# kzampog/cilantro

Hardware: AMD Instinct MI355X
Metric: ICP corr. pairs/sec (+ iterations/sec), synthetic uniform clouds (higher is better)
Workload: dtype f32 search / f64 accumulate+solve

## Files before the change

### cilantro_amd/capi.py

```python
import ctypes as C
import os

_HERE = os.path.dirname(os.path.abspath(__file__))
LIB_PATH = os.environ.get("CILHIP_LIB_PATH") or os.path.join(_HERE, "lib", "libcilantro_hip.so")

OK, ERR_INVALID, ERR_HIP, ERR_UNSUPPORTED, ERR_NO_DEVICE = 0, -1, -2, -3, -4
MEM_HOST, MEM_DEVICE = 0, 1
METRIC_POINT_TO_POINT, METRIC_COMBINED = 0, 1
SUMS_LEN = 48
NONE_IDX = 0xFFFFFFFF

SYMBOLS = [
    "cilhip_create", "cilhip_destroy", "cilhip_last_error", "cilhip_set_stream", "cilhip_synchronize",
    "cilhip_set_target", "cilhip_set_source", "cilhip_set_source_normals", "cilhip_get_means", "cilhip_set_color_features", "cilhip_share_target", "cilhip_find_correspondences",
    "cilhip_get_nn", "cilhip_get_correspondences", "cilhip_estimate_point_to_point",
    "cilhip_estimate_combined", "cilhip_estimate_affine", "cilhip_icp_default_params", "cilhip_icp_run", "cilhip_icp_begin",
    "cilhip_icp_partial_sums", "cilhip_icp_apply_sums", "cilhip_icp_state", "cilhip_compute_residuals",
    "cilhip_get_grid_info", "cilhip_get_last_timing", "cilhip_enable_kernel_timing", "cilhip_prepare_source", "cilhip_get_last_run_forms", "cilhip_get_last_warm_iterations", "cilhip_get_last_matches_origin", "cilhip_get_matches_transform", "cilhip_get_last_form_timing", "cilhip_get_last_iteration_timing", "cilhip_get_last_run_trace", "cilhip_estimate_combined_two_sets", "cilhip_icp_run_two_sets", "cilhip_set_pair_weight_callback", "cilhip_kmeans_set_pruning", "cilhip_get_tie_count", "cilhip_get_tie_rule_stats", "cilhip_get_tie_order_info", "cilhip_build_tie_order", "cilhip_tie_order_create", "cilhip_tie_order_destroy", "cilhip_tie_order_tables", "cilhip_load_tie_order", "cilhip_multi_create", "cilhip_multi_destroy", "cilhip_multi_last_error", "cilhip_multi_context", "cilhip_multi_set_clouds", "cilhip_multi_icp_run", "cilhip_multi_repartitions", "cilhip_multi_last_host_time", "cilhip_multi_set_slab_slack", "cilhip_multi_shard_sizes", "cilhip_rank_comm_unique_id", "cilhip_rank_comm_prepare", "cilhip_rank_comm_init", "cilhip_rank_comm_destroy", "cilhip_icp_iterate_ranked", "cilhip_get_last_allreduce_timing", "cilhip_get_last_host_enqueue_time", "cilhip_set_slab_guard", "cilhip_get_slab_violation", "cilhip_get_slab_violation_state",
    "cilhip_set_option", "cilhip_option_count", "cilhip_option_info", "cilhip_set_option_id", "cilhip_get_option", "cilhip_get_last_timing2", "cilhip_set_shard_info", "cilhip_icp_partial_keys",
    "cilhip_icp_sums_from_keys", "cilhip_icp_order_keys", "cilhip_icp_sums_from_ordered_keys", "cilhip_debug_counters", "cilhip_kmeans3f", "cilhip_kmeans3f_assign", "cilhip_kmeans3f_ex", "cilhip_kmeans3f_assign_ex", "cilhip_kmeans_shard_create", "cilhip_kmeans_shard_destroy", "cilhip_kmeans_shard_maxabs", "cilhip_kmeans_scale_exponent", "cilhip_kmeans_shard_assign", "cilhip_kmeans_shard_farthest", "cilhip_kmeans_shard_move_point", "cilhip_kmeans_shard_labels",
    "cilhip_plane_ransac3f", "cilhip_plane_score3f", "cilhip_plane_fit3f", "cilhip_transform_ransac3f", "cilhip_transform_score3f", "cilhip_transform_fit3f", "cilhip_knn3f", "cilhip_knn_set_tie_rule", "cilhip_normals_knn3f", "cilhip_normals_radius3f", "cilhip_radius_search3f",
]


PAIR_WEIGHT_FN = C.CFUNCTYPE(None, C.c_void_p, C.POINTER(C.c_uint64), C.POINTER(C.c_uint64), C.POINTER(C.c_float), C.c_size_t,
                             C.POINTER(C.c_float), C.POINTER(C.c_float))


class IcpParams(C.Structure):
    _fields_ = [
        ("metric", C.c_int), ("w_p2p", C.c_float), ("w_p2pl", C.c_float), ("max_iter", C.c_size_t),
        ("conv_tol", C.c_float), ("max_opt_iter", C.c_size_t), ("opt_conv_tol", C.c_float),
        ("max_sq_dist", C.c_float),
    ]


class IcpResult(C.Structure):
    _fields_ = [
        ("T", C.c_float * 16), ("iterations", C.c_size_t), ("last_delta_norm", C.c_float),
        ("last_ncorr", C.c_size_t),
    ]


class GridInfo(C.Structure):
    _fields_ = [
        ("nx", C.c_int), ("ny", C.c_int), ("nz", C.c_int), ("cell", C.c_float),
        ("origin", C.c_float * 3), ("n_cells", C.c_size_t), ("avg_occupancy", C.c_double),
        ("build_ms", C.c_double),
    ]


class OptionInfo(C.Structure):
    _fields_ = [("id", C.c_int), ("key", C.c_char_p), ("default_value", C.c_double), ("min_value", C.c_double), ("max_value", C.c_double),
                ("doc", C.c_char_p)]


class TieOrderInfo(C.Structure):
    _fields_ = [("loaded", C.c_int), ("builds", C.c_int), ("build_ms", C.c_double), ("pending", C.c_size_t)]


class PlaneModel(C.Structure):
    _fields_ = [
        ("normal", C.c_float * 3), ("offset", C.c_float), ("iterations", C.c_size_t), ("n_inliers", C.c_size_t),
        ("target_reached", C.c_int), ("device_ms", C.c_double),
    ]


class TransformModel(C.Structure):
    _fields_ = [
        ("T", C.c_float * 16), ("iterations", C.c_size_t), ("n_inliers", C.c_size_t), ("have_model", C.c_int),
        ("target_reached", C.c_int), ("device_ms", C.c_double),
    ]


_lib = None


def load():
    global _lib
    if _lib is not None:
        return _lib
    if not os.path.exists(LIB_PATH):
        raise RuntimeError(
            f"{LIB_PATH} is missing: the HIP extension has not been built "
            "(run `python -m cilantro_amd.build` / `__graft_entry__.build()`). There is no CPU fallback."
        )
    try:
        import torch
    except ImportError:
        pass
    L = C.CDLL(LIB_PATH)
    vp, f32p, f64p = C.c_void_p, C.c_void_p, C.c_void_p
    L.cilhip_create.argtypes = [C.POINTER(vp), C.c_int]
    L.cilhip_destroy.argtypes = [vp]
    L.cilhip_destroy.restype = None
    L.cilhip_last_error.argtypes = [vp]
    L.cilhip_last_error.restype = C.c_char_p
    L.cilhip_set_stream.argtypes = [vp, vp]
    L.cilhip_synchronize.argtypes = [vp]
    L.cilhip_set_target.argtypes = [vp, f32p, f32p, C.c_size_t, C.c_int]
    L.cilhip_set_source.argtypes = [vp, f32p, C.c_size_t, C.c_int]
    L.cilhip_set_source_normals.argtypes = [vp, f32p, C.c_int]
    L.cilhip_get_means.argtypes = [vp, f32p, f32p]
    L.cilhip_find_correspondences.argtypes = [vp, f32p, C.c_float, C.POINTER(C.c_size_t)]
    L.cilhip_get_nn.argtypes = [vp, vp, f32p, C.c_int]
    L.cilhip_get_correspondences.argtypes = [vp, vp, vp, f32p, C.c_size_t, C.POINTER(C.c_size_t)]
    L.cilhip_estimate_point_to_point.argtypes = [vp, f32p, f64p, C.POINTER(C.c_int)]
    L.cilhip_estimate_combined.argtypes = [vp, C.c_float, C.c_float, C.c_size_t, C.c_float, f32p, f64p,
                                           f64p, C.POINTER(C.c_int)]
    L.cilhip_estimate_affine.argtypes = [vp, C.c_float, C.c_float, C.c_int, f32p, f64p, f64p, C.POINTER(C.c_size_t), C.POINTER(C.c_int)]
    L.cilhip_icp_default_params.argtypes = [C.POINTER(IcpParams)]
    L.cilhip_icp_default_params.restype = None
    L.cilhip_icp_run.argtypes = [vp, C.POINTER(IcpParams), f32p, C.POINTER(IcpResult)]
    L.cilhip_icp_begin.argtypes = [vp, C.POINTER(IcpParams), f32p, f32p]
    L.cilhip_icp_partial_sums.argtypes = [vp, f64p]
    L.cilhip_icp_apply_sums.argtypes = [vp, f64p]
    L.cilhip_icp_state.argtypes = [vp, C.POINTER(IcpResult)]
    L.cilhip_compute_residuals.argtypes = [vp, C.c_int, C.c_float, C.c_float, f32p, f32p, C.c_int]
    L.cilhip_get_grid_info.argtypes = [vp, C.POINTER(GridInfo)]
    L.cilhip_get_last_timing.argtypes = [vp, C.POINTER(C.c_double), C.POINTER(C.c_double), C.POINTER(C.c_int)]
    L.cilhip_enable_kernel_timing.argtypes = [vp, C.c_int]
    L.cilhip_set_option.argtypes = [vp, C.c_char_p, C.c_double]
    L.cilhip_share_target.argtypes = [vp, vp]
    L.cilhip_option_count.argtypes = []
    L.cilhip_option_info.argtypes = [C.c_int]
    L.cilhip_option_info.restype = C.POINTER(OptionInfo)
    L.cilhip_set_option_id.argtypes = [vp, C.c_int, C.c_double]
    L.cilhip_get_option.argtypes = [vp, C.c_char_p, C.POINTER(C.c_double)]
    L.cilhip_set_shard_info.argtypes = [vp, C.c_uint64, f32p, f32p]
    L.cilhip_icp_partial_keys.argtypes = [vp, vp]
    L.cilhip_debug_counters.argtypes = [vp, vp]
    L.cilhip_kmeans3f.argtypes = [C.c_int, f32p, C.c_size_t, C.c_int, f32p, C.c_size_t, C.c_size_t, C.c_float, vp, C.POINTER(C.c_size_t)]
    L.cilhip_kmeans3f_assign.argtypes = [C.c_int, f32p, C.c_size_t, C.c_int, f32p, C.c_size_t, vp]
    L.cilhip_kmeans3f_ex.argtypes = [C.c_int, f32p, C.c_size_t, C.c_int, f32p, C.c_size_t, C.c_size_t, C.c_float, C.c_int, vp, C.POINTER(C.c_size_t)]
    L.cilhip_kmeans3f_assign_ex.argtypes = [C.c_int, f32p, C.c_size_t, C.c_int, f32p, C.c_size_t, C.c_int, vp]
    L.cilhip_kmeans_shard_create.argtypes = [C.c_int, f32p, C.c_size_t, C.c_int, C.c_size_t, C.c_uint64, C.POINTER(C.c_void_p)]
    L.cilhip_kmeans_shard_destroy.argtypes = [vp]
    L.cilhip_kmeans_shard_destroy.restype = None
    L.cilhip_kmeans_shard_maxabs.argtypes = [vp, C.POINTER(C.c_float)]
    L.cilhip_kmeans_scale_exponent.argtypes = [C.c_double, C.c_size_t]
    L.cilhip_kmeans_shard_assign.argtypes = [vp, vp, C.c_int, C.c_int, vp, C.POINTER(C.c_uint64)]
    L.cilhip_kmeans_shard_farthest.argtypes = [vp, C.c_uint32, vp, C.POINTER(C.c_uint64)]
    L.cilhip_kmeans_shard_move_point.argtypes = [vp, C.c_uint64, C.c_uint32, vp]
    L.cilhip_kmeans_shard_labels.argtypes = [vp, vp]
    L.cilhip_plane_ransac3f.argtypes = [C.c_int, f32p, C.c_size_t, C.c_int, vp, C.c_uint64, C.c_float, C.c_size_t, C.c_size_t,
                                        C.c_int, C.POINTER(PlaneModel), vp, vp]
    L.cilhip_plane_score3f.argtypes = [C.c_int, f32p, C.c_size_t, C.c_int, f32p, C.c_size_t, C.c_float, vp]
    L.cilhip_plane_fit3f.argtypes = [C.c_int, f32p, C.c_size_t, C.c_int, f32p]
    L.cilhip_transform_ransac3f.argtypes = [C.c_int, f32p, f32p, C.c_size_t, C.c_int, vp, C.c_uint64, C.c_float, C.c_size_t, C.c_size_t,
                                            C.c_int, C.POINTER(TransformModel), vp, vp]
    L.cilhip_transform_score3f.argtypes = [C.c_int, f32p, f32p, C.c_size_t, C.c_int, f32p, C.c_size_t, C.c_float, vp]
    L.cilhip_transform_fit3f.argtypes = [C.c_int, f32p, f32p, C.c_size_t, C.c_int, f32p]
    L.cilhip_knn3f.argtypes = [C.c_int, f32p, C.c_size_t, f32p, C.c_size_t, C.c_int, C.c_size_t, C.c_float, vp, vp, vp]
    L.cilhip_normals_radius3f.argtypes = [C.c_int, f32p, C.c_size_t, C.c_int, C.c_float, f32p, f32p, f32p]
    L.cilhip_radius_search3f.argtypes = [C.c_int, f32p, C.c_size_t, f32p, C.c_size_t, C.c_int, C.c_float, vp, vp, vp, C.c_size_t,
                                         C.POINTER(C.c_size_t)]
    L.cilhip_normals_knn3f.argtypes = [C.c_int, f32p, C.c_size_t, C.c_int, C.c_size_t, C.c_float, f32p, f32p, f32p]
    L.cilhip_icp_sums_from_keys.argtypes = [vp, vp, f64p]
    L.cilhip_icp_order_keys.argtypes = [vp, vp, vp]
    L.cilhip_icp_sums_from_ordered_keys.argtypes = [vp, vp, vp, f64p]
    L.cilhip_get_last_timing2.argtypes = [vp, C.POINTER(C.c_double), C.POINTER(C.c_double)]
    L.cilhip_prepare_source.argtypes = [vp, C.c_void_p, C.c_int, C.POINTER(C.c_double)]
    L.cilhip_get_last_run_forms.argtypes = [vp, C.POINTER(C.c_int), C.POINTER(C.c_int)]
    L.cilhip_get_last_warm_iterations.argtypes = [vp, C.POINTER(C.c_int)]
    L.cilhip_set_color_features.argtypes = [vp, vp, vp, C.c_int]
    L.cilhip_get_last_matches_origin.argtypes = [vp, C.POINTER(C.c_int)]
    L.cilhip_get_matches_transform.argtypes = [vp, vp]
    L.cilhip_get_last_form_timing.argtypes = [vp, C.c_int, C.POINTER(C.c_double), C.POINTER(C.c_int)]
    L.cilhip_estimate_combined_two_sets.argtypes = [vp, vp, C.c_float, C.c_float, C.c_size_t, C.c_float, vp, C.POINTER(C.c_int)]
    L.cilhip_icp_run_two_sets.argtypes = [vp, C.c_float, vp, C.c_float, C.POINTER(IcpParams), vp, C.POINTER(IcpResult)]
    L.cilhip_set_pair_weight_callback.argtypes = [vp, PAIR_WEIGHT_FN, vp]
    L.cilhip_get_tie_count.argtypes = [vp, vp, C.c_float, C.POINTER(C.c_size_t)]
    L.cilhip_get_last_iteration_timing.argtypes = [vp, C.c_int, C.POINTER(C.c_int), vp, vp]
    L.cilhip_get_tie_rule_stats.argtypes = [vp, C.POINTER(C.c_size_t), C.POINTER(C.c_size_t)]
    L.cilhip_get_tie_order_info.argtypes = [vp, C.POINTER(TieOrderInfo)]
    L.cilhip_build_tie_order.argtypes = [vp]
    L.cilhip_tie_order_create.argtypes = [vp, C.c_size_t, C.POINTER(C.c_void_p)]
    L.cilhip_tie_order_tables.argtypes = [vp, vp, vp, vp, C.c_size_t, C.POINTER(C.c_size_t), C.POINTER(C.c_int)]
    L.cilhip_tie_order_destroy.argtypes = [vp]
    L.cilhip_tie_order_destroy.restype = None
    L.cilhip_load_tie_order.argtypes = [vp, vp, vp]
    L.cilhip_multi_create.argtypes = [C.POINTER(vp), C.POINTER(C.c_int), C.c_int]
    L.cilhip_multi_destroy.argtypes = [vp]; L.cilhip_multi_destroy.restype = None
    L.cilhip_multi_last_error.argtypes = [vp]; L.cilhip_multi_last_error.restype = C.c_char_p
    L.cilhip_multi_context.argtypes = [vp, C.c_int]; L.cilhip_multi_context.restype = vp
    L.cilhip_multi_set_clouds.argtypes = [vp, vp, vp, C.c_size_t, vp, C.c_size_t, C.c_float, C.c_int, vp]
    L.cilhip_multi_icp_run.argtypes = [vp, C.POINTER(IcpParams), vp, C.c_int, C.POINTER(IcpResult)]
    L.cilhip_multi_repartitions.argtypes = [vp]
    L.cilhip_multi_set_slab_slack.argtypes = [vp, C.c_float]
    L.cilhip_multi_shard_sizes.argtypes = [vp, C.c_int, C.POINTER(C.c_size_t), C.POINTER(C.c_size_t)]
    L.cilhip_rank_comm_unique_id.argtypes = [vp]
    L.cilhip_rank_comm_init.argtypes = [vp, vp, C.c_int, C.c_int]
    L.cilhip_rank_comm_prepare.argtypes = [vp]
    L.cilhip_rank_comm_destroy.argtypes = [vp]
    L.cilhip_icp_iterate_ranked.argtypes = [vp, C.c_int]
    L.cilhip_get_last_allreduce_timing.argtypes = [vp, C.POINTER(C.c_double), C.POINTER(C.c_int)]
    L.cilhip_get_last_host_enqueue_time.argtypes = [vp, C.POINTER(C.c_double)]
    L.cilhip_get_last_run_trace.argtypes = [vp, C.c_int, C.POINTER(C.c_int), C.POINTER(C.c_uint), C.POINTER(C.c_uint), C.POINTER(C.c_float), C.POINTER(C.c_float), C.POINTER(C.c_int)]
    L.cilhip_set_slab_guard.argtypes = [vp, C.c_int, C.c_float, f32p, f32p, f32p]
    L.cilhip_get_slab_violation.argtypes = [vp, C.POINTER(C.c_int)]
    L.cilhip_get_slab_violation_state.argtypes = [vp, C.POINTER(C.c_int), vp]
    for name in SYMBOLS:
        fn = getattr(L, name)
        if name not in ("cilhip_destroy", "cilhip_last_error", "cilhip_icp_default_params", "cilhip_option_info"):
            fn.restype = C.c_int
    _lib = L
    return L


class CilhipError(RuntimeError):
    def __init__(self, code, msg):
        super().__init__(f"cilhip error {code}: {msg}")
        self.code = code

# ... 9 lines not shown
```

### cilantro_amd/csrc/c_api.hip

```cpp
#include "../../include/cilantro_hip/c_api.h"

#include <hip/hip_runtime.h>

#include <algorithm>
#include <atomic>
#include <chrono>
#include <condition_variable>
#include <mutex>
#include <cmath>
#include <cstddef>
#include <cstdio>
#include <cstring>
#include <new>
#include <string>
#include <thread>
#include <vector>

#include "internal.hpp"

using namespace cilhip;

struct TargetShare { int refs = 0; std::vector<void*> allocs; };

struct cilhip_ctx {
  int device = 0;
  TargetShare* tshare = nullptr;
  hipStream_t own_stream = nullptr;
  hipStream_t stream = nullptr;
  std::string err;

  bool has_target = false;
  GridDev grid{};
  bool has_normals = false;
  double grid_occ = 0.0;
  size_t grid_cells = 0;
  double build_ms = 0.0;
  float dst_mean[3] = {0, 0, 0};
  uint32_t index_offset = 0;
  bool partial_target = false;
  uint32_t* d_inv_perm = nullptr;

  bool has_source = false;
  uint32_t ns = 0;
  float* d_src_xyz = nullptr;
  float4* d_src_sorted = nullptr;
  SortWorkspace sort_ws;
  uint32_t tile_aux_cap = 0;
  uint2* d_tiles = nullptr;
  float4* d_tile_center = nullptr;
  int* d_tile_box = nullptr;
  float tile_axes[9] = {0, 0, 0, 0, 0, 0, 0, 0, 0};
  unsigned long long* d_defer_mask = nullptr;
  uint32_t* d_defer_flag = nullptr;
  uint32_t* d_unproven = nullptr;
  bool warm_banned = false;
  Feedback* h_feedback = nullptr;
  Feedback* d_feedback = nullptr;
  unsigned int run_tag = 0;
  bool far_mode = true;
  int last_fused_iters = 0, last_two_pass_iters = 0, last_warm_iters = 0;
  int run_calls = 0;
  bool run_warm_on = false;
  unsigned int run_judged = 0;
  std::vector<unsigned char> iter_form;
  std::vector<unsigned char> trace_form;
  double form_ms[5] = {0, 0, 0, 0, 0};
  int form_n[5] = {0, 0, 0, 0, 0};
  int warm_start = 1;
  uint32_t* d_dbg = nullptr;
  uint4* d_trace = nullptr;
  uint32_t ntiles = 0;
  int tiled = 1;
  bool src_sorted = false;
  float sort_T[16];
  float src_mean[3] = {0, 0, 0};
  float* d_src_nrm = nullptr;
  float4* d_src_nrm_sorted = nullptr;
  uint32_t* d_nn_pos = nullptr;
  float* d_nn_d2 = nullptr;
  float4* d_warm_rec = nullptr;
  bool rec_valid = false;
  bool src3_valid = false;
  float* d_nn_lb = nullptr;
  bool lb_fresh = false;
  bool warm_forecast = true;
  int tie_rule = 2;
  uint2* d_tief_leaf_slot = nullptr;
  uint4* d_tief_nodes = nullptr;
  int tief_builds = 0;
  uint2* d_tie_leaf_slot = nullptr;
  uint4* d_tie_nodes = nullptr;
  unsigned int* d_tie_counters = nullptr;
  unsigned int* d_ticket = nullptr;
  int group_lanes = -1;
  double wait_us = 0.0;
  bool feat_warm = true;
  bool affine_device_loop = true;
  bool fused_epilogue = false;
  unsigned int tie_counters_host[4] = {0, 0, 0, 0};
  bool tie_counters_fresh = false;
  double tie_build_ms = 0.0;
  int tie_builds = 0;
  bool rev_tie_aware = false;
  uint2* d_rev_tie_leaf_slot = nullptr;
  uint4* d_rev_tie_nodes = nullptr;
  size_t rev_tie_nodes_cap = 0;
  bool rev_tie_valid = false;
  float rev_tie_T[16];
  int rev_tie_builds = 0;
  float warm_extra = 0.0625f;
  bool pair_records = true;
  void* rank_comm = nullptr; int rank_comm_size = 0; double* d_rank_sums = nullptr;
  bool tile_records = true;
  float warm_enter = 0.15f;
  float warm_thresh = 0.0f;
  int warm_strikes = 0;
  float src_center[3] = {0, 0, 0}, src_half[3] = {0, 0, 0};
  float* d_safe2 = nullptr;
  int cw_point_kind = 0, cw_plane_kind = 0;
  float cw_point_sigma = 1.0f, cw_plane_sigma = 1.0f;
  cilhip_pair_weight_fn weight_fn = nullptr;
  void* weight_user = nullptr;
  float* d_wtab = nullptr;
// ... 54 lines not shown

  cilhip_icp_params run_prm{};
  bool run_active = false;
  int guard_axis = -1;
  float guard_slack = 0.0f, guard_center[3] = {0, 0, 0}, guard_half[3] = {0, 0, 0}, guard_T[16] = {0};
  float run_src_mean[3] = {0, 0, 0};

  bool kernel_timing = false;
  int timing_stride = 1;
  std::vector<unsigned int> timed_iter;
  std::vector<float> timed_ms;
  double last_loop_ms = 0.0, last_search_ms = 0.0, last_acc_ms = 0.0;
  int last_search_launches = 0;
  size_t run_nev = 0;
  std::vector<hipEvent_t> ev, ev_acc;
  std::vector<hipEvent_t> ev_ar;
  size_t run_nar = 0;
  double last_allreduce_ms = 0.0; int last_allreduce_n = 0;
  double run_enqueue_us = 0.0; int run_enqueue_iters = 0;

};

#define CK(ctx, call)                                                                                   \
  do {                                                                                                  \
    hipError_t e_ = (call);                                                                             \
    if (e_ != hipSuccess) {                                                                             \
      (ctx)->err = std::string(#call) + ": " + hipGetErrorString(e_);                                   \
      return CILHIP_ERR_HIP;                                                                            \
    }                                                                                                   \
  } while (0)

static int fail(cilhip_ctx* c, int code, const char* msg) {
  if (c) c->err = msg;
  return code;
}

static const float kIdentity[16] = {1, 0, 0, 0, 0, 1, 0, 0, 0, 0, 1, 0, 0, 0, 0, 1};
namespace cilhip {
hipStream_t ctx_stream(const cilhip_ctx* c) { return c->stream; }
double ctx_wait_us(const cilhip_ctx* c) { return c->wait_us; }
}

static void drop_src_grid(cilhip_ctx* c) {
  if (c->has_src_grid) { free_grid(c->src_grid); c->has_src_grid = false; }
  if (c->d_src_safe2) { (void)hipFree(c->d_src_safe2); c->d_src_safe2 = nullptr; }
  if (c->d_grid_to_sorted) { (void)hipFree(c->d_grid_to_sorted); c->d_grid_to_sorted = nullptr; }
  if (c->d_src_rgb_grid) { (void)hipFree(c->d_src_rgb_grid); c->d_src_rgb_grid = nullptr; }
}
static void drop_matches(cilhip_ctx* c) { c->have_nn = false; c->d2_stale = false; c->pending_matches = false; c->matches_origin = 0; }
static void drop_rev_tie_tables(cilhip_ctx* c) {
  if (c->d_rev_tie_leaf_slot) { (void)hipFree(c->d_rev_tie_leaf_slot); c->d_rev_tie_leaf_slot = nullptr; }
  if (c->d_rev_tie_nodes) { (void)hipFree(c->d_rev_tie_nodes); c->d_rev_tie_nodes = nullptr; }
  c->rev_tie_nodes_cap = 0; c->rev_tie_valid = false; c->rev_tie_aware = false;
}
static void target_ptr_free(cilhip_ctx* c, const void* p) {
  if (!p) return;
  if (c->tshare && std::find(c->tshare->allocs.begin(), c->tshare->allocs.end(), p) != c->tshare->allocs.end()) return;
  (void)hipFree(const_cast<void*>(p));
}
static void release_target_share(cilhip_ctx* c) {
  if (!c->tshare) return;
  if (--c->tshare->refs == 0) {
    for (void* p : c->tshare->allocs) (void)hipFree(p);
    delete c->tshare;
  }
  c->tshare = nullptr;
}
static void drop_feat_tie_tables(cilhip_ctx* c) {
  if (c->d_tief_leaf_slot) { (void)hipFree(c->d_tief_leaf_slot); c->d_tief_leaf_slot = nullptr; }
  if (c->d_tief_nodes) { (void)hipFree(c->d_tief_nodes); c->d_tief_nodes = nullptr; }
}
static void drop_tie_tables(cilhip_ctx* c) {
  target_ptr_free(c, c->d_tie_leaf_slot); c->d_tie_leaf_slot = nullptr;
  target_ptr_free(c, c->d_tie_nodes); c->d_tie_nodes = nullptr;
}
static void release_target(cilhip_ctx* c) {
  if (c->has_target) {
    target_ptr_free(c, c->grid.pts); target_ptr_free(c, c->grid.nrm); target_ptr_free(c, c->grid.pn); target_ptr_free(c, c->grid.cell_start);
    c->grid.pts = nullptr; c->grid.nrm = nullptr; c->grid.pn = nullptr; c->grid.cell_start = nullptr;
    c->has_target = false;
  }
  target_ptr_free(c, c->d_inv_perm); c->d_inv_perm = nullptr;
  target_ptr_free(c, c->d_safe2); c->d_safe2 = nullptr;
  drop_tie_tables(c);
  drop_feat_tie_tables(c);
  release_target_share(c);
}

extern "C" {

int cilhip_create(cilhip_ctx** out, int device) {
  if (!out) return CILHIP_ERR_INVALID;
  *out = nullptr;
  int ndev = 0;
  if (hipGetDeviceCount(&ndev) != hipSuccess || ndev <= 0) return CILHIP_ERR_NO_DEVICE;
  if (device < 0 || device >= ndev) return CILHIP_ERR_INVALID;
  cilhip_ctx* c = new (std::nothrow) cilhip_ctx();
  if (!c) return CILHIP_ERR_HIP;
  c->device = device;
  if (hipSetDevice(device) != hipSuccess || hipStreamCreateWithFlags(&c->own_stream, hipStreamNonBlocking) != hipSuccess) {
    delete c;
    return CILHIP_ERR_HIP;
  }
  c->stream = c->own_stream;
  if (hipMalloc(&c->d_state, sizeof(IcpState)) != hipSuccess || hipMalloc(&c->d_count, sizeof(unsigned long long)) != hipSuccess ||
      hipMalloc(&c->d_defer_flag, sizeof(uint32_t)) != hipSuccess || hipMemset(c->d_defer_flag, 0, sizeof(uint32_t)) != hipSuccess ||
      hipMalloc(&c->d_unproven, 128 * sizeof(uint32_t)) != hipSuccess || hipMemset(c->d_unproven, 0, 128 * sizeof(uint32_t)) != hipSuccess ||
      hipMalloc(&c->d_ticket, sizeof(unsigned int)) != hipSuccess || hipMemset(c->d_ticket, 0, sizeof(unsigned int)) != hipSuccess ||
      hipHostMalloc(&c->h_feedback, sizeof(Feedback), hipHostMallocMapped | hipHostMallocCoherent) != hipSuccess ||
      hipHostGetDevicePointer(reinterpret_cast<void**>(&c->d_feedback), c->h_feedback, 0) != hipSuccess ||
      hipMalloc(&c->d_trace, RUN_TRACE_CAP * sizeof(uint4)) != hipSuccess || hipMemset(c->d_trace, 0, RUN_TRACE_CAP * sizeof(uint4)) != hipSuccess ||
      hipMalloc(&c->d_stage, REDUCE_STAGE_DOUBLES * sizeof(double)) != hipSuccess || hipMalloc(&c->d_sums, 3 * SUMS_MAX * sizeof(double)) != hipSuccess) {
    delete c;
    return CILHIP_ERR_HIP;
  }
  if (hipMemset(c->d_state, 0, sizeof(IcpState)) != hipSuccess) { delete c; return CILHIP_ERR_HIP; }
  c->d_tie_counters = reinterpret_cast<unsigned int*>(reinterpret_cast<char*>(c->d_state) + offsetof(IcpState, tie_counters));
  memcpy(c->sort_T, kIdentity, sizeof(kIdentity));
  memcpy(c->nn_T, kIdentity, sizeof(kIdentity));
  *out = c;
  return CILHIP_OK;
}

static void free_source(cilhip_ctx* c) {
  drop_rev_tie_tables(c);
  if (c->d_src_xyz) (void)hipFree(c->d_src_xyz);
  if (c->d_src_sorted) (void)hipFree(c->d_src_sorted);
  if (c->d_nn_pos) (void)hipFree(c->d_nn_pos);
  if (c->d_nn_d2) (void)hipFree(c->d_nn_d2);
  if (c->d_warm_rec) { (void)hipFree(c->d_warm_rec); c->d_warm_rec = nullptr; }
  if (c->d_nn_lb) { (void)hipFree(c->d_nn_lb); c->d_nn_lb = nullptr; }
  c->src3_valid = false; c->lb_fresh = false;
  c->rec_valid = false;
  if (c->d_out_idx) (void)hipFree(c->d_out_idx);
  if (c->d_out_d2) (void)hipFree(c->d_out_d2);
  free_sort_workspace(c->sort_ws);
  c->tile_aux_cap = 0;
  if (c->d_tile_box) (void)hipFree(c->d_tile_box);
  if (c->d_src_nrm) (void)hipFree(c->d_src_nrm);
  if (c->d_src_nrm_sorted) (void)hipFree(c->d_src_nrm_sorted);
  c->d_src_nrm = nullptr; c->d_src_nrm_sorted = nullptr;
  if (c->d_src_rgb) (void)hipFree(c->d_src_rgb);
  if (c->d_src_rgb_sorted) (void)hipFree(c->d_src_rgb_sorted);
  c->d_src_rgb = nullptr; c->d_src_rgb_sorted = nullptr;
  if (c->d_defer_mask) (void)hipFree(c->d_defer_mask);
  if (c->d_keys) (void)hipFree(c->d_keys);
  c->d_keys = nullptr;
  if (c->d_own_order) (void)hipFree(c->d_own_order);
  c->d_own_order = nullptr;
  c->d_tiles = nullptr; c->d_tile_center = nullptr; c->d_tile_box = nullptr; c->ntiles = 0; c->d_defer_mask = nullptr;
  c->d_src_xyz = nullptr; c->d_src_sorted = nullptr; c->d_nn_pos = nullptr; c->d_nn_d2 = nullptr;
  c->d_out_idx = nullptr; c->d_out_d2 = nullptr;
  drop_src_grid(c);
  if (c->d_src_inv) { (void)hipFree(c->d_src_inv); c->d_src_inv = nullptr; }
  if (c->d_grid_to_sorted) { (void)hipFree(c->d_grid_to_sorted); c->d_grid_to_sorted = nullptr; }
  c->has_source = false; c->src_sorted = false; drop_matches(c); c->ns = 0;
  c->have_pairs = false; c->pairs.count = 0;
  c->far_mode = true;
  c->warm_banned = false;
}

void cilhip_destroy(cilhip_ctx* c) {
  if (!c) return;
  (void)hipSetDevice(c->device);
  (void)hipStreamSynchronize(c->stream);
  (void)cilhip_rank_comm_destroy(c);
  free_source(c);
  release_target(c);
  if (c->d_ticket) (void)hipFree(c->d_ticket);
  if (c->d_wtab) (void)hipFree(c->d_wtab);
  if (c->d_wtab_in) (void)hipFree(c->d_wtab_in);
  if (c->d_dst_rgb) (void)hipFree(c->d_dst_rgb);
  if (c->d_dst_rgb_sorted) (void)hipFree(c->d_dst_rgb_sorted);
  if (c->d_state) (void)hipFree(c->d_state);
  if (c->d_state_id) (void)hipFree(c->d_state_id);
  free_pairs(c->pairs);
  if (c->d_partials) (void)hipFree(c->d_partials);
  if (c->d_sel_state) (void)hipFree(c->d_sel_state);
  if (c->d_winner) (void)hipFree(c->d_winner);
  if (c->d_count) (void)hipFree(c->d_count);
  if (c->d_dbg) (void)hipFree(c->d_dbg);
  if (c->d_trace) (void)hipFree(c->d_trace);
  if (c->d_defer_flag) (void)hipFree(c->d_defer_flag);
  if (c->d_unproven) (void)hipFree(c->d_unproven);
  if (c->d_rev_pos) (void)hipFree(c->d_rev_pos);
  if (c->d_rev_d2) (void)hipFree(c->d_rev_d2);
  if (c->h_feedback) (void)hipHostFree(c->h_feedback);
  if (c->d_stage) (void)hipFree(c->d_stage);
  if (c->d_sums) (void)hipFree(c->d_sums);
  for (auto e : c->ev) (void)hipEventDestroy(e);
  for (auto e : c->ev_acc) (void)hipEventDestroy(e);
  for (auto e : c->ev_ar) (void)hipEventDestroy(e);

  if (c->own_stream) (void)hipStreamDestroy(c->own_stream);
  delete c;
}

const char* cilhip_last_error(const cilhip_ctx* c) { return c ? c->err.c_str() : "null context"; }

int cilhip_set_stream(cilhip_ctx* c, void* s) {
  if (!c) return CILHIP_ERR_INVALID;
  (void)hipSetDevice(c->device);
  (void)hipStreamSynchronize(c->stream);
  c->stream = s ? (hipStream_t)s : c->own_stream;
  return CILHIP_OK;
}

int cilhip_synchronize(cilhip_ctx* c) {
  if (!c) return CILHIP_ERR_INVALID;
  CK(c, hipSetDevice(c->device));
  CK(c, hipStreamSynchronize(c->stream));
  return CILHIP_OK;
}

namespace {
struct OptionRow { cilhip_option_info_t info; double (*get)(const cilhip_ctx*); };
#define OPT(ID, KEY, DEF, LO, HI, DOC, EXPR) {{ID, KEY, DEF, LO, HI, DOC}, [](const cilhip_ctx* c) -> double { return (double)(EXPR); }}
const OptionRow g_options[] = {
  OPT(CILHIP_OPT_FUSED, "fused", 0, 0, 1, "1 = one per-lane search+accumulate kernel per iteration; 0 = search kernel + streaming accumulation (or the LDS tiles)", c->fused),
  OPT(CILHIP_OPT_INLIER_FRACTION, "inlier_fraction", 1, 0, 1, "CorrespondenceSearchKDTree::setInlierFraction: keep that fraction of the correspondences, nearest first", c->inlier_fraction),
  OPT(CILHIP_OPT_ONE_TO_ONE, "one_to_one", 0, 0, 1, "setOneToOne: a target point keeps only its nearest source point", c->one_to_one),
  OPT(CILHIP_OPT_TILED, "tiled", 1, 0, 2, "LDS-tiled search: 0 = never, 1 = when the cloud fills the chip with full tiles, 2 = always", c->tiled),
  OPT(CILHIP_OPT_WARM_START, "warm_start", 1, 0, 2, "warm-started iterations (margin proof): 0 = never, 1 = when the loop is near alignment, 2 = from the second iteration on", c->warm_start),
  OPT(CILHIP_OPT_WARM_FORECAST, "warm_forecast", 1, 0, 1, "the cold kernels' forecast gates the warm-started form (0: the step alone; tests)", c->warm_forecast),
  OPT(CILHIP_OPT_FUSED_EPILOGUE, "fused_epilogue", 0, 0, 1, "stage-1 reduction + epilogue as one launch behind a device-scope fence (bitwise equal, measured slower; A/B)", c->fused_epilogue),
  OPT(CILHIP_OPT_GROUP_SEARCH, "group_search", -1, -1, 64, "lanes per query of the cooperative global-memory search: -1 = the loop decides, 0 = never, 4 / 8 / 16 / 32 / 64", c->group_lanes),
  OPT(CILHIP_OPT_TIE_RULE, "tie_rule", 2, 0, 2, "exactly equidistant nearest points: 0 = lowest index, 1 = the reference's kd-tree order (tables up front), 2 = the same, tables when a tie is first met", c->tie_rule),
  OPT(CILHIP_OPT_WARM_EXTRA_FRACTION, "warm_extra_fraction", 0.0625, 1e-9, 1, "room (fraction of a cell) of the ball a warm-started iteration searches a listed query in", c->warm_extra),
  OPT(CILHIP_OPT_PAIR_RECORDS, "pair_records", 1, 0, 1, "streaming accumulation gathers a match's point and normal from one 32-byte record (A/B)", c->pair_records),
  OPT(CILHIP_OPT_TILE_RECORDS, "tile_records", 1, 0, 1, "the accumulating tile kernel writes the warm-started form's match records itself (A/B)", c->tile_records),
  OPT(CILHIP_OPT_WARM_ENTER_FRACTION, "warm_enter_fraction", 0.15, 1e-9, 1e9, "the warm-started form is entered once an update moves no source point by more than this fraction of a cell", c->warm_enter),
  OPT(CILHIP_OPT_POINT_WEIGHT_EVALUATOR, "point_weight_evaluator", 0, 0, 2, "combined metric, point-to-point terms: 0 = UnityWeightEvaluator, 1 = DistanceEvaluator, 2 = RBFKernelWeightEvaluator", c->cw_point_kind),
  OPT(CILHIP_OPT_PLANE_WEIGHT_EVALUATOR, "plane_weight_evaluator", 0, 0, 2, "combined metric, point-to-plane terms: 0 = Unity, 1 = Identity (distance), 2 = RBF kernel", c->cw_plane_kind),
  OPT(CILHIP_OPT_POINT_WEIGHT_SIGMA, "point_weight_sigma", 1, 1e-30, 1e30, "sigma of the RBF evaluator of the point-to-point terms", c->cw_point_sigma),
  OPT(CILHIP_OPT_PLANE_WEIGHT_SIGMA, "plane_weight_sigma", 1, 1e-30, 1e30, "sigma of the RBF evaluator of the point-to-plane terms", c->cw_plane_sigma),
  OPT(CILHIP_OPT_TILE_ACCUMULATION, "tile_accumulation", 1, 0, 2, "first Gauss-Newton step accumulated inside the LDS tiles: 0 = never, 1 = unless the source is far from alignment, 2 = always", (c->tile_acc ? (c->tile_acc_adaptive ? 1 : 2) : 0)),
  OPT(CILHIP_OPT_SEARCH_DIRECTION, "search_direction", 0, 0, 2, "CorrespondenceSearchDirection: 0 = SECOND_TO_FIRST, 1 = FIRST_TO_SECOND, 2 = BOTH", c->search_dir),
  OPT(CILHIP_OPT_FEATURE_NORMAL_WEIGHT, "feature_normal_weight", 0, 0, 1e30, "PointNormalFeaturesAdaptor's normal weight (> 0: the search runs on 6-D features)", c->normal_weight),
  OPT(CILHIP_OPT_FEATURE_KIND, "feature_kind", 0, 0, 2, "second feature block: 0 = normals (follow the transform), 1 = colours (do not), 2 = normals + colours (9-D)", c->feature_kind),
  OPT(CILHIP_OPT_FEATURE_COLOR_WEIGHT, "feature_color_weight", 0, 0, 1e30, "PointNormalColorFeaturesAdaptor's colour weight (feature_kind 2)", c->color_weight),
  OPT(CILHIP_OPT_SYMMETRIC_METRIC, "symmetric_metric", 1, 0, 1, "source normals, when set, switch the combined metric to the symmetric objective", c->symmetric),
  OPT(CILHIP_OPT_TRANSFORM_MODE, "transform_mode", 0, 0, 1, "ICP instance family: 0 = rigid, 1 = affine", c->transform_mode),
  OPT(CILHIP_OPT_REQUIRE_RECIPROCALITY, "require_reciprocality", 0, 0, 1, "setRequireReciprocality (search_direction BOTH)", c->reciprocal),
  OPT(CILHIP_OPT_CELL_OCCUPANCY, "cell_occupancy", 1, 1e-3, 1e6, "target points per grid cell the next cilhip_set_target aims at", c->cell_occupancy),
  OPT(CILHIP_OPT_REFINED_OCCUPANCY_FACTOR, "refined_occupancy_factor", 3, 1, 64, "how much denser than that a grid that had to be refined (surface, clusters) may stay", c->refined_occupancy),
  OPT(CILHIP_OPT_KERNEL_TIMING, "kernel_timing", 0, 0, 1, "hipEvents around the search / accumulation kernels (cilhip_enable_kernel_timing)", c->kernel_timing),
  OPT(CILHIP_OPT_KERNEL_TIMING_STRIDE, "kernel_timing_stride", 1, 1, 4096, "with kernel timing on: iterations 0..2 and every stride-th one carry events", c->timing_stride),
  OPT(CILHIP_OPT_REVERSE_WARM_START, "reverse_warm_start", 1, 0, 1, "device-resident FIRST_TO_SECOND / BOTH loops: reverse searches after the first start from the previous reverse matches (margin test over the source; A/B)", c->reverse_warm),
  OPT(CILHIP_OPT_FEATURE_WARM_START, "feature_warm_start", 1, 0, 1, "feature adaptors (SECOND_TO_FIRST loops): searches warm-started from the previous matches once the loop moves little (margin test with the feature distance; A/B)", c->feat_warm),
  OPT(CILHIP_OPT_AFFINE_DEVICE_LOOP, "affine_device_loop", 1, 0, 1, "affine classes: 1 = device-resident loop (one-pass moments, solve in the epilogue kernel), 0 = host-driven loop (three passes + host solve; A/B)", c->affine_device_loop),
};
#undef OPT
constexpr int N_OPTIONS = (int)(sizeof(g_options) / sizeof(g_options[0]));
static_assert(N_OPTIONS == CILHIP_OPT_COUNT, "one table row per enum cilhip_option value, in the enum's order");
}

int cilhip_option_count(void) { return N_OPTIONS; }
const cilhip_option_info_t* cilhip_option_info(int id) { return (id >= 0 && id < N_OPTIONS) ? &g_options[id].info : nullptr; }
int cilhip_set_option_id(cilhip_ctx* c, cilhip_option id, double value) {
  if (!c) return CILHIP_ERR_INVALID;
  if ((int)id < 0 || (int)id >= N_OPTIONS) return fail(c, CILHIP_ERR_INVALID, "set_option_id: unknown option");
  return cilhip_set_option(c, g_options[(int)id].info.key, value);
}
int cilhip_get_option(cilhip_ctx* c, const char* key, double* value) {
  if (!c || !key || !value) return CILHIP_ERR_INVALID;
  for (int i = 0; i < N_OPTIONS; ++i)
    if (!strcmp(key, g_options[i].info.key)) { *value = g_options[i].get(c); return CILHIP_OK; }
  return fail(c, CILHIP_ERR_INVALID, "get_option: unknown key");
}

int cilhip_set_option(cilhip_ctx* c, const char* key, double value) {
  if (!c || !key) return CILHIP_ERR_INVALID;
  if (value != value) return fail(c, CILHIP_ERR_INVALID, "set_option: the value is not a number");
  if (!strcmp(key, "fused")) { c->fused = value != 0.0; return CILHIP_OK; }
  if (!strcmp(key, "inlier_fraction")) { if (c->inlier_fraction != value && c->pending_matches) drop_matches(c); c->inlier_fraction = value; return CILHIP_OK; }
  if (!strcmp(key, "one_to_one")) { if (c->one_to_one != (value != 0.0) && c->pending_matches) drop_matches(c); c->one_to_one = value != 0.0; return CILHIP_OK; }
  if (!strcmp(key, "tiled")) { c->tiled = (int)value; return CILHIP_OK; }
  if (!strcmp(key, "warm_start")) { c->warm_start = (int)value; return CILHIP_OK; }
  if (!strcmp(key, "warm_forecast")) { c->warm_forecast = value != 0.0; return CILHIP_OK; }
  if (!strcmp(key, "fused_epilogue")) { c->fused_epilogue = value != 0.0; return CILHIP_OK; }
  if (!strcmp(key, "reverse_warm_start")) { c->reverse_warm = value != 0.0; return CILHIP_OK; }
  if (!strcmp(key, "feature_warm_start")) { c->feat_warm = value != 0.0; return CILHIP_OK; }
  if (!strcmp(key, "affine_device_loop")) { c->affine_device_loop = value != 0.0; return CILHIP_OK; }
  if (!strcmp(key, "group_search")) {
    if (value != -1.0 && value != 0.0 && value != 4.0 && value != 8.0 && value != 16.0 && value != 32.0 && value != 64.0)
      return fail(c, CILHIP_ERR_INVALID, "group_search: -1 (the loop decides), 0 (never), or 4, 8, 16, 32, 64 lanes per query");
    c->group_lanes = (int)value;
    return CILHIP_OK;
  }
  if (!strcmp(key, "tie_rule")) {
    if (value != 0.0 && value != 1.0 && value != 2.0)
      return fail(c, CILHIP_ERR_INVALID, "tie_rule: 0 (lowest index), 1 (the reference's kd-tree order, tables built up front) or 2 (the same, tables built when a tie is first met)");
    if (((int)value != 0) != (c->tie_rule != 0)) drop_matches(c);
    c->tie_rule = (int)value;
    return CILHIP_OK;
  }
  if (!strcmp(key, "warm_extra_fraction")) {
    if (!(value > 0.0 && value <= 1.0)) return fail(c, CILHIP_ERR_INVALID, "warm_extra_fraction: in (0, 1]");
    c->warm_extra = (float)value;
    return CILHIP_OK;
  }
  if (!strcmp(key, "pair_records")) { c->pair_records = value != 0.0; return CILHIP_OK; }
  if (!strcmp(key, "tile_records")) { c->tile_records = value != 0.0; return CILHIP_OK; }
  if (!strcmp(key, "warm_enter_fraction")) {
    if (!(value > 0.0)) return fail(c, CILHIP_ERR_INVALID, "warm_enter_fraction: > 0 (fraction of a grid cell)");
    c->warm_enter = (float)value;
    return CILHIP_OK;
  }
  if (!strcmp(key, "point_weight_evaluator") || !strcmp(key, "plane_weight_evaluator")) {
    if (value != 0.0 && value != 1.0 && value != 2.0) return fail(c, CILHIP_ERR_INVALID, "weight evaluator: 0 = Unity, 1 = Identity, 2 = RBF kernel");
    (key[1] == 'o' ? c->cw_point_kind : c->cw_plane_kind) = (int)value;
    return CILHIP_OK;
  }
  if (!strcmp(key, "point_weight_sigma") || !strcmp(key, "plane_weight_sigma")) {
    if (!(value > 0.0)) return fail(c, CILHIP_ERR_INVALID, "weight evaluator sigma must be positive");
    (key[1] == 'o' ? c->cw_point_sigma : c->cw_plane_sigma) = (float)value;
    return CILHIP_OK;
  }
  if (!strcmp(key, "tile_accumulation")) { c->tile_acc = value != 0.0; c->tile_acc_adaptive = value != 2.0; return CILHIP_OK; }
  if (!strcmp(key, "search_direction")) {
    if (value != 0.0 && value != 1.0 && value != 2.0) return fail(c, CILHIP_ERR_INVALID, "search_direction: 0 = SECOND_TO_FIRST, 1 = FIRST_TO_SECOND, 2 = BOTH");
    c->search_dir = (int)value; drop_matches(c); c->have_pairs = false;
    return CILHIP_OK;
  }
  if (!strcmp(key, "feature_normal_weight")) {
    if (!(value >= 0.0)) return fail(c, CILHIP_ERR_INVALID, "feature_normal_weight: >= 0 (0 = plain point features)");
    if (c->normal_weight != (float)value) drop_feat_tie_tables(c);
    c->normal_weight = (float)value; drop_matches(c); c->have_pairs = false;
    return CILHIP_OK;
  }
  if (!strcmp(key, "feature_kind")) {
    if (value != 0.0 && value != 1.0 && value != 2.0)
      return fail(c, CILHIP_ERR_INVALID, "feature_kind: 0 = normals (follow the transform), 1 = colours (do not), 2 = normals + colours (9-D)");
    if ((int)value != c->feature_kind) { drop_src_grid(c); drop_feat_tie_tables(c); }
    c->feature_kind = (int)value; drop_matches(c); c->have_pairs = false;
    return CILHIP_OK;
  }
  if (!strcmp(key, "feature_color_weight")) {
    if (!(value >= 0.0)) return fail(c, CILHIP_ERR_INVALID, "feature_color_weight: >= 0");
    if (c->color_weight != (float)value) drop_feat_tie_tables(c);
    c->color_weight = (float)value; drop_matches(c); c->have_pairs = false;
    return CILHIP_OK;
  }
  if (!strcmp(key, "symmetric_metric")) { c->symmetric = value != 0.0; return CILHIP_OK; }
  if (!strcmp(key, "transform_mode")) {
    if (value != 0.0 && value != 1.0) return fail(c, CILHIP_ERR_INVALID, "transform_mode: 0 = rigid, 1 = affine");
    c->transform_mode = (int)value;
    return CILHIP_OK;
  }
  if (!strcmp(key, "require_reciprocality")) { c->reciprocal = value != 0.0; drop_matches(c); c->have_pairs = false; return CILHIP_OK; }
  if (!strcmp(key, "cell_occupancy")) { c->cell_occupancy = value; return CILHIP_OK; }
  if (!strcmp(key, "refined_occupancy_factor")) {
    if (!(value >= 1.0 && value <= 64.0)) return fail(c, CILHIP_ERR_INVALID, "refined_occupancy_factor: in [1, 64]");
    c->refined_occupancy = value;
    return CILHIP_OK;
  }
  if (!strcmp(key, "kernel_timing")) { c->kernel_timing = value != 0.0; return CILHIP_OK; }
  if (!strcmp(key, "kernel_timing_stride")) {
    if (!(value >= 1.0 && value <= 4096.0)) return fail(c, CILHIP_ERR_INVALID, "kernel_timing_stride: 1 .. 4096");
    c->timing_stride = (int)value;
    return CILHIP_OK;
  }
  return fail(c, CILHIP_ERR_INVALID, "set_option: unknown key");
}

int cilhip_debug_counters(cilhip_ctx* c, uint32_t out[2]) {
  if (!c || !out) return CILHIP_ERR_INVALID;
  out[0] = out[1] = 0;
  if (!c->d_defer_mask || !c->ntiles) return CILHIP_OK;
  CK(c, hipSetDevice(c->device));
  if (!c->d_dbg) CK(c, hipMalloc(&c->d_dbg, 2 * sizeof(uint32_t)));
  launch_count_deferred(c->d_defer_mask, c->ntiles, c->d_dbg, c->stream);
  CK(c, hipMemcpyAsync(out, c->d_dbg, 2 * sizeof(uint32_t), hipMemcpyDeviceToHost, c->stream));
  CK(c, hipStreamSynchronize(c->stream));
#ifdef CILHIP_EXP_PHASE_CLOCKS
  cilhip::debug_dump_phase_clocks();
#endif
  return CILHIP_OK;
}

int cilhip_get_last_timing2(cilhip_ctx* c, double* search_ms, double* accumulate_ms) {
  if (!c) return CILHIP_ERR_INVALID;
  if (search_ms) *search_ms = c->last_search_ms;
  if (accumulate_ms) *accumulate_ms = c->last_acc_ms;
  return CILHIP_OK;
}

int cilhip_get_last_iteration_timing(cilhip_ctx* c, int cap, int* n, unsigned int* iteration, float* kernel_ms) {
  if (!c || !n || cap < 0) return CILHIP_ERR_INVALID;
  const size_t m = c->timed_ms.size() < c->timed_iter.size() ? c->timed_ms.size() : c->timed_iter.size();
  *n = (int)m;
  for (size_t k = 0; k < m && k < (size_t)cap; ++k) { if (iteration) iteration[k] = c->timed_iter[k]; if (kernel_ms) kernel_ms[k] = c->timed_ms[k]; }
  return CILHIP_OK;
}

int cilhip_get_last_form_timing(cilhip_ctx* c, int form, double* kernel_ms, int* launches) {
  if (!c || form < 0 || form > 4) return CILHIP_ERR_INVALID;
  if (kernel_ms) *kernel_ms = c->form_ms[form];
  if (launches) *launches = c->form_n[form];
  return CILHIP_OK;
}

int cilhip_get_last_run_trace(cilhip_ctx* c, int cap, int* n_out, unsigned int* unproven, unsigned int* listed, float* step, float* delta, int* form) {
  if (!c || !n_out || cap < 0) return CILHIP_ERR_INVALID;
  CK(c, hipSetDevice(c->device));
  IcpState hs;
  CK(c, hipMemcpyAsync(&hs, c->d_state, sizeof(hs), hipMemcpyDeviceToHost, c->stream));
  uint4 tr[RUN_TRACE_CAP];
  CK(c, hipMemcpyAsync(tr, c->d_trace, sizeof(tr), hipMemcpyDeviceToHost, c->stream));
  CK(c, hipStreamSynchronize(c->stream));
  const int n = std::min(std::min(hs.iterations, (int)RUN_TRACE_CAP), cap);
  for (int i = 0; i < n; ++i) {
    if (unproven) unproven[i] = tr[i].x;
    if (listed) listed[i] = tr[i].y;
    if (step) memcpy(&step[i], &tr[i].z, 4);
    if (delta) memcpy(&delta[i], &tr[i].w, 4);
    if (form) form[i] = (size_t)i < c->trace_form.size() ? (int)(c->trace_form[i] & 0x7f) : -1;
  }
  *n_out = n;
  return CILHIP_OK;
}

int cilhip_get_last_warm_iterations(cilhip_ctx* c, int* warm_iterations) {
  if (!c || !warm_iterations) return CILHIP_ERR_INVALID;
  *warm_iterations = c->last_warm_iters;
  return CILHIP_OK;
}

int cilhip_get_last_run_forms(cilhip_ctx* c, int* one_pass_iterations, int* two_pass_iterations) {
  if (!c) return CILHIP_ERR_INVALID;
  if (one_pass_iterations) *one_pass_iterations = c->last_fused_iters;
  if (two_pass_iterations) *two_pass_iterations = c->last_two_pass_iters;
  return CILHIP_OK;
}

int cilhip_enable_kernel_timing(cilhip_ctx* c, int on) {
  if (!c) return CILHIP_ERR_INVALID;
  c->kernel_timing = on != 0;
  return CILHIP_OK;
}

static int upload(cilhip_ctx* c, const float* src, size_t count, int mem, float** d_out) {
  *d_out = nullptr;
  CK(c, hipMalloc(d_out, (count ? count : 1) * sizeof(float)));
  if (count)
    CK(c, hipMemcpyAsync(*d_out, src, count * sizeof(float), mem == CILHIP_MEM_DEVICE ? hipMemcpyDeviceToDevice : hipMemcpyHostToDevice, c->stream));
  return CILHIP_OK;
}

int cilhip_set_target(cilhip_ctx* c, const float* xyz, const float* nrm, size_t n, int mem) {
  if (!c) return CILHIP_ERR_INVALID;
  if ((n && !xyz) || n >= 0xFFFFFFF0ull) return fail(c, CILHIP_ERR_INVALID, "set_target: bad cloud (null or >= 2^32-16 points)");
  CK(c, hipSetDevice(c->device));
  auto t0 = std::chrono::steady_clock::now();
  release_target(c);
  if (c->d_winner) { (void)hipFree(c->d_winner); c->d_winner = nullptr; }
  if (c->d_rev_pos) { (void)hipFree(c->d_rev_pos); c->d_rev_pos = nullptr; }
  if (c->d_rev_d2) { (void)hipFree(c->d_rev_d2); c->d_rev_d2 = nullptr; }
  float *d_xyz = nullptr, *d_nrm = nullptr;
  int rc = upload(c, xyz, 3 * n, mem, &d_xyz);
  if (rc) return rc;
  if (nrm) { rc = upload(c, nrm, 3 * n, mem, &d_nrm); if (rc) { (void)hipFree(d_xyz); return rc; } }
  GridBuildResult r{};
  double mean[3];
  hipError_t e = build_grid(d_xyz, d_nrm, (uint32_t)n, c->stream, &r, mean, c->cell_occupancy, c->refined_occupancy);
  (void)hipFree(d_xyz);
  if (d_nrm) (void)hipFree(d_nrm);
  if (e != hipSuccess) { c->err = std::string("build_grid: ") + hipGetErrorString(e); return CILHIP_ERR_HIP; }
  c->grid = r.grid; c->grid_occ = r.avg_occupancy; c->grid_cells = r.n_cells;
  c->warm_banned = false;
  c->dst_rgb_sorted_ok = false;
  if (c->d_dst_rgb) { (void)hipFree(c->d_dst_rgb); c->d_dst_rgb = nullptr; }
  if (c->d_dst_rgb_sorted) { (void)hipFree(c->d_dst_rgb_sorted); c->d_dst_rgb_sorted = nullptr; }
  c->has_normals = (nrm != nullptr);
  for (int i = 0; i < 3; ++i) c->dst_mean[i] = (float)mean[i];
  c->partial_target = false;
  c->has_target = true;
  c->src_sorted = false;
  drop_matches(c);
  c->have_pairs = false; c->pairs.count = 0;
  c->far_mode = true;
  c->build_ms = std::chrono::duration<double, std::milli>(std::chrono::steady_clock::now() - t0).count();
  return CILHIP_OK;
}

int cilhip_share_target(cilhip_ctx* c, cilhip_ctx* from) {
  if (!c || !from || c == from) return CILHIP_ERR_INVALID;
  if (!from->has_target) return fail(c, CILHIP_ERR_INVALID, "share_target: the other context has no target");
  if (c->device != from->device) return fail(c, CILHIP_ERR_INVALID, "share_target: the two contexts live on different devices");
  CK(c, hipSetDevice(c->device));
  CK(c, hipStreamSynchronize(from->stream));
  CK(c, hipStreamSynchronize(c->stream));
  release_target(c);
  if (c->d_winner) { (void)hipFree(c->d_winner); c->d_winner = nullptr; }
  if (c->d_rev_pos) { (void)hipFree(c->d_rev_pos); c->d_rev_pos = nullptr; }
  if (c->d_rev_d2) { (void)hipFree(c->d_rev_d2); c->d_rev_d2 = nullptr; }
  if (c->d_dst_rgb) { (void)hipFree(c->d_dst_rgb); c->d_dst_rgb = nullptr; }
  if (c->d_dst_rgb_sorted) { (void)hipFree(c->d_dst_rgb_sorted); c->d_dst_rgb_sorted = nullptr; }
  c->dst_rgb_sorted_ok = false;
  if (!from->tshare) { from->tshare = new (std::nothrow) TargetShare(); if (!from->tshare) return fail(c, CILHIP_ERR_HIP, "share_target: out of memory"); from->tshare->refs = 1; }
  TargetShare* sh = from->tshare;
  const void* ptrs[] = {from->grid.pts, from->grid.nrm, from->grid.pn, from->grid.cell_start, from->d_inv_perm, from->d_safe2, from->d_tie_leaf_slot, from->d_tie_nodes};
  for (const void* p : ptrs)
    if (p && std::find(sh->allocs.begin(), sh->allocs.end(), p) == sh->allocs.end()) sh->allocs.push_back(const_cast<void*>(p));
  ++sh->refs;
  c->tshare = sh;
  c->grid = from->grid; c->has_target = true; c->has_normals = from->has_normals;
  c->grid_occ = from->grid_occ; c->grid_cells = from->grid_cells; c->build_ms = 0.0;
  for (int i = 0; i < 3; ++i) c->dst_mean[i] = from->dst_mean[i];
  c->index_offset = from->index_offset; c->partial_target = from->partial_target;
  c->d_inv_perm = from->d_inv_perm; c->d_safe2 = from->d_safe2;
  c->d_tie_leaf_slot = from->d_tie_leaf_slot; c->d_tie_nodes = from->d_tie_nodes;
  c->warm_banned = false;
  c->src_sorted = false;
  drop_matches(c);
  c->have_pairs = false; c->pairs.count = 0;
  c->far_mode = true;
  return CILHIP_OK;
}

int cilhip_set_source(cilhip_ctx* c, const float* xyz, size_t n, int mem) {
  if (!c) return CILHIP_ERR_INVALID;
  if ((n && !xyz) || n >= 0xFFFFFFF0ull) return fail(c, CILHIP_ERR_INVALID, "set_source: bad cloud");
  CK(c, hipSetDevice(c->device));
  free_source(c);
  int rc = upload(c, xyz, 3 * n, mem, &c->d_src_xyz);
  if (rc) return rc;
  const size_t cap = n ? n : 1;
  CK(c, hipMalloc(&c->d_src_sorted, cap * sizeof(float4)));
  CK(c, hipMalloc(&c->d_nn_pos, cap * sizeof(uint32_t)));
  CK(c, hipMalloc(&c->d_nn_d2, cap * sizeof(float)));
  c->ns = (uint32_t)n;
  double mean[3];
  float lo[3], hi[3];
  hipError_t e = mean3_device(c->d_src_xyz, c->ns, c->stream, mean, lo, hi);
  if (e != hipSuccess) { c->err = std::string("mean3: ") + hipGetErrorString(e); return CILHIP_ERR_HIP; }
  for (int i = 0; i < 3; ++i) {
    c->src_mean[i] = (float)mean[i];
    c->src_center[i] = 0.5f * (lo[i] + hi[i]);
    c->src_half[i] = c->ns ? std::max(hi[i] - c->src_center[i], c->src_center[i] - lo[i]) * 1.000001f : 0.0f;
    if (!(c->src_half[i] >= 0.0f) || !std::isfinite(c->src_center[i])) { c->src_center[i] = 0.0f; c->src_half[i] = 1.0e30f; }
  }
  const int nb = std::max(iter_num_blocks(c->ns), warm_num_blocks(c->ns));
  if (nb > c->partial_blocks) {
    if (c->d_partials) (void)hipFree(c->d_partials);
    CK(c, hipMalloc(&c->d_partials, (size_t)nb * SUMS_MAX * sizeof(double)));
    c->partial_blocks = nb;
  }
  c->has_source = true;
  return CILHIP_OK;
}

int cilhip_set_source_normals(cilhip_ctx* c, const float* nrm, int mem) {
  if (!c) return CILHIP_ERR_INVALID;
  if (!c->has_source) return fail(c, CILHIP_ERR_INVALID, "set_source_normals: set_source first");
  CK(c, hipSetDevice(c->device));
  if (c->d_src_nrm) { (void)hipFree(c->d_src_nrm); c->d_src_nrm = nullptr; }
  if (c->d_src_nrm_sorted) { (void)hipFree(c->d_src_nrm_sorted); c->d_src_nrm_sorted = nullptr; }
  c->have_pairs = false; c->pairs.count = 0;
  drop_src_grid(c);
  if (!nrm) return CILHIP_OK;
  int rc = upload(c, nrm, 3 * (size_t)c->ns, mem, &c->d_src_nrm);
  if (rc) return rc;
  c->src_nrm0[0] = c->src_nrm0[1] = c->src_nrm0[2] = 0.0f;
  if (c->ns) {
    CK(c, hipMemcpyAsync(c->src_nrm0, c->d_src_nrm, 3 * sizeof(float), hipMemcpyDeviceToHost, c->stream));
    CK(c, hipStreamSynchronize(c->stream));
  }
  CK(c, hipMalloc(&c->d_src_nrm_sorted, (c->ns ? c->ns : 1) * sizeof(float4)));
  c->src_sorted = false;
  drop_matches(c);
  c->have_pairs = false; c->pairs.count = 0;
  return CILHIP_OK;
}

int cilhip_set_color_features(cilhip_ctx* c, const float* dst_rgb, const float* src_rgb, int mem) {
  if (!c) return CILHIP_ERR_INVALID;
  if (!c->has_target || !c->has_source) return fail(c, CILHIP_ERR_INVALID, "set_color_features: set_target and set_source first");
  if (!dst_rgb || !src_rgb) return fail(c, CILHIP_ERR_INVALID, "set_color_features: both clouds' colours are needed");
  CK(c, hipSetDevice(c->device));
  if (c->d_dst_rgb) { (void)hipFree(c->d_dst_rgb); c->d_dst_rgb = nullptr; }
  if (c->d_src_rgb) { (void)hipFree(c->d_src_rgb); c->d_src_rgb = nullptr; }
  if (c->d_src_rgb_sorted) { (void)hipFree(c->d_src_rgb_sorted); c->d_src_rgb_sorted = nullptr; }
  int rc = upload(c, dst_rgb, 3 * (size_t)c->grid.n, mem, &c->d_dst_rgb);
  if (rc) return rc;
  rc = upload(c, src_rgb, 3 * (size_t)c->ns, mem, &c->d_src_rgb);
  if (rc) return rc;
  CK(c, hipMalloc(&c->d_src_rgb_sorted, (c->ns ? c->ns : 1) * sizeof(float4)));
  c->dst_rgb_sorted_ok = false;
  c->src_sorted = false;
  drop_src_grid(c);
  drop_feat_tie_tables(c);
  drop_matches(c);
  c->have_pairs = false; c->pairs.count = 0;
  return CILHIP_OK;
}

int cilhip_get_means(cilhip_ctx* c, float dm[3], float sm[3]) {
  if (!c) return CILHIP_ERR_INVALID;
  if (dm) memcpy(dm, c->dst_mean, sizeof(c->dst_mean));
  if (sm) memcpy(sm, c->src_mean, sizeof(c->src_mean));
  return CILHIP_OK;
}

static int ensure_sorted(cilhip_ctx* c, const float T[16]) {
  if (!c->has_target || !c->has_source) return fail(c, CILHIP_ERR_INVALID, "set_target and set_source first");
  bool need = !c->src_sorted;
  if (!need) {
    float a[3], b[3];
    transform_point(T, c->src_mean[0], c->src_mean[1], c->src_mean[2], a[0], a[1], a[2]);
    transform_point(c->sort_T, c->src_mean[0], c->src_mean[1], c->src_mean[2], b[0], b[1], b[2]);
    float dl = 0.f;
    for (int i = 0; i < 3; ++i) dl = fmaxf(dl, fabsf(a[i] - b[i]));
    float dr = 0.f;
    for (int i = 0; i < 11; ++i) if (i % 4 != 3) dr = fmaxf(dr, fabsf(T[i] - c->sort_T[i]));
    const float ext = fmaxf(c->grid.nx, fmaxf(c->grid.ny, c->grid.nz)) * c->grid.cell;
    if (dl > 4.0f * c->grid.cell || dr * ext > 4.0f * c->grid.cell) need = true;
  }
  if (need) {
    c->d_tiles = nullptr; c->d_tile_center = nullptr; c->ntiles = 0;
    hipError_t e = sort_source(c->d_src_xyz, c->ns, c->grid, T, c->d_src_sorted, c->stream, &c->d_tiles, &c->d_tile_center, c->tile_axes, &c->ntiles, &c->sort_ws);
    if (e != hipSuccess) { c->err = std::string("sort_source: ") + hipGetErrorString(e); return CILHIP_ERR_HIP; }
    if (c->ntiles + 1 > c->tile_aux_cap) {
      if (c->d_tile_box) { (void)hipFree(c->d_tile_box); c->d_tile_box = nullptr; }
      if (c->d_defer_mask) { (void)hipFree(c->d_defer_mask); c->d_defer_mask = nullptr; }
      c->tile_aux_cap = 0;
      const uint32_t cap = c->ntiles + 1 + c->ntiles / 8;
      CK(c, hipMalloc(&c->d_defer_mask, (size_t)cap * 2 * (TILE_THREADS / 64) * sizeof(unsigned long long)));
      CK(c, hipMalloc(&c->d_tile_box, (size_t)cap * 8 * sizeof(int)));
      c->tile_aux_cap = cap;
    }
    CK(c, hipMemsetAsync(c->d_defer_mask, 0, ((size_t)c->ntiles + 1) * 2 * (TILE_THREADS / 64) * sizeof(unsigned long long), c->stream));
    {
      const int rows = std::max(std::max(iter_num_blocks(c->ns), warm_num_blocks(c->ns)), tiled_partial_rows(c->ntiles));
      if (rows > c->partial_blocks) {
        if (c->d_partials) (void)hipFree(c->d_partials);
        c->d_partials = nullptr; c->partial_blocks = 0;
        CK(c, hipMalloc(&c->d_partials, (size_t)rows * SUMS_MAX * sizeof(double)));
        c->partial_blocks = rows;
      }
    }
    if (c->d_src_nrm) launch_gather_by_w(c->d_src_sorted, c->d_src_nrm, c->ns, c->d_src_nrm_sorted, c->stream);
    if (c->d_src_rgb) launch_gather_by_w(c->d_src_sorted, c->d_src_rgb, c->ns, c->d_src_rgb_sorted, c->stream);
    if (c->d_src_inv) { (void)hipFree(c->d_src_inv); c->d_src_inv = nullptr; }
    if (c->d_grid_to_sorted) { (void)hipFree(c->d_grid_to_sorted); c->d_grid_to_sorted = nullptr; }
    memcpy(c->sort_T, T, sizeof(c->sort_T));
    c->src_sorted = true;
    c->src3_valid = false; c->rec_valid = false; c->lb_fresh = false;
    drop_matches(c);
  }
  return CILHIP_OK;
}

int cilhip_prepare_source(cilhip_ctx* c, const float* T, int force, double* ms) {
  if (!c) return CILHIP_ERR_INVALID;
  CK(c, hipSetDevice(c->device));
  CK(c, hipStreamSynchronize(c->stream));
  const auto t0 = std::chrono::steady_clock::now();
  if (force) c->src_sorted = false;
  const int rc = ensure_sorted(c, T ? T : kIdentity);
  if (rc) return rc;
  CK(c, hipStreamSynchronize(c->stream));
  if (ms) *ms = std::chrono::duration<double, std::milli>(std::chrono::steady_clock::now() - t0).count();
  return CILHIP_OK;
}

static bool use_tiled(const cilhip_ctx* c) {
  if (c->ns >= 0x80000000ull) return false;
  if (c->tiled >= 2) return true;
  if (c->tiled != 1 || c->ntiles < 600) return false;
  const double fill = (double)c->ns / ((double)c->ntiles * (double)TILE_QUERIES);
  const double region_cells = (double)(CUBE_EDGE + 3) * (CUBE_EDGE + 3) * (CUBE_EDGE + 3);
  const double density = c->grid_occ > 1.0 ? c->grid_occ - 1.0 : c->grid_occ;
  return fill >= 0.45 && density * region_cells <= 0.92 * (double)TILE_CAP;
}

static bool filters_active(const cilhip_ctx* c) {
  return (c->inlier_fraction > 0.0 && c->inlier_fraction < 1.0) || c->one_to_one;
}

enum { FORM_SEARCH = 0, FORM_TILE_ONE_PASS = 1, FORM_WARM_FIRST = 2, FORM_WARM = 3, FORM_LANE_FUSED = 4 };
static void warm_run_reset(cilhip_ctx* c) { c->warm_thresh = c->warm_enter * c->grid.cell; c->warm_strikes = 0; }
static bool warm_keeps_paying(cilhip_ctx* c, unsigned int listed) {
  if ((unsigned long long)listed * 4ull <= (unsigned long long)c->ns) return true;
  c->warm_thresh *= 0.5f;
  if (++c->warm_strikes >= 3) c->warm_banned = true;
  return false;
}
static bool warm_worthwhile(const cilhip_ctx* c, float step) { return step < c->warm_thresh; }
static int ensure_warm_buffers(cilhip_ctx* c) {
  const size_t cap = c->ns ? c->ns : 1;
  if (!c->d_warm_rec) { CK(c, hipMalloc(&c->d_warm_rec, cap * (sizeof(float4) + 2 * sizeof(F3)))); c->src3_valid = false; }
  if (!c->d_nn_lb) CK(c, hipMalloc(&c->d_nn_lb, cap * sizeof(float)));
  if (!c->src3_valid) {
    launch_copy_src3(c->d_src_sorted, c->ns, reinterpret_cast<F3*>(c->d_warm_rec + cap) + cap, c->stream);
    c->src3_valid = true;
  }
  return CILHIP_OK;
}
static void ensure_pair_records(cilhip_ctx* c) {
  if (c->grid.pn || !c->pair_records || !c->grid.nrm || !c->grid.n) return;
  float4* pn = nullptr;
  if (hipMalloc(&pn, (size_t)c->grid.n * 2 * sizeof(float4)) != hipSuccess) { (void)hipGetLastError(); return; }
  launch_interleave_pn(c->grid.pts, c->grid.nrm, c->grid.n, pn, c->stream);
  c->grid.pn = pn;
// ... 207 lines not shown
    *again = true;
    CK(c, hipMemsetAsync(c->d_tie_counters, 0, 4 * sizeof(unsigned int), c->stream));
    return build_feat_tie_tables(c);
  }
  if (!tie_mode_on(c) || c->partial_target || !c->ns || !c->grid.n) return CILHIP_OK;
  const bool fwd_open = !c->d_tie_leaf_slot && c->search_dir != 1;
  const bool rev_open = !c->rev_tie_aware && c->search_dir != 0;
  if (!fwd_open && !rev_open) return CILHIP_OK;
  unsigned int cnt[4];
  if (c->tie_counters_fresh) {
    memcpy(cnt, c->tie_counters_host, sizeof(cnt));
  } else {
    const int rc = read_tie_counters(c, cnt);
    if (rc) return rc;
  }
  c->tie_counters_fresh = false;
  const bool fwd = fwd_open && cnt[0] != 0u, rev = rev_open && cnt[3] >= 16u && (unsigned long long)cnt[3] * 100000ull >= (unsigned long long)c->grid.n;
  if (!fwd && !rev) return CILHIP_OK;
  *again = true;
  CK(c, hipMemsetAsync(c->d_tie_counters, 0, 4 * sizeof(unsigned int), c->stream));
  if (rev) c->rev_tie_aware = true;
  return fwd ? build_tie_tables(c) : CILHIP_OK;
}

static int apply_filters(cilhip_ctx* c) {
  if (!filters_active(c) || c->ns == 0) return CILHIP_OK;
  if (c->inlier_fraction > 0.0 && c->inlier_fraction < 1.0) {
    if (!c->d_keys) CK(c, hipMalloc(&c->d_keys, (size_t)c->ns * sizeof(unsigned long long)));
    if (!c->d_sel_state) CK(c, hipMalloc(&c->d_sel_state, filter_state_bytes()));
    launch_filter_fraction(c->d_src_sorted, c->d_nn_pos, c->d_nn_d2, c->ns, c->inlier_fraction, c->d_keys, c->d_sel_state, c->stream);
  }
  if (c->one_to_one && c->grid.n) {
    if (!c->d_winner) CK(c, hipMalloc(&c->d_winner, (size_t)c->grid.n * sizeof(unsigned long long)));
    launch_filter_one_to_one(c->d_src_sorted, c->d_nn_pos, c->d_nn_d2, c->ns, c->d_winner, c->grid.n, c->stream);
  }
  CK(c, hipGetLastError());
  return CILHIP_OK;
}

static FeatSpec feat_spec_of(const cilhip_ctx* c) {
  FeatSpec f{};
  f.w = c->normal_weight;
  f.enabled = feat6(c) ? 1 : 0;
  if (c->feature_kind == 1) { f.src = c->d_src_rgb_sorted; f.dst = c->d_dst_rgb_sorted; f.mode = 2; }
  else { f.src = c->d_src_nrm ? c->d_src_nrm_sorted : nullptr; f.dst = c->grid.nrm; f.mode = c->transform_mode == 1 ? 1 : 0; }
  if (c->feature_kind == 2) { f.src2 = c->d_src_rgb_sorted; f.dst2 = c->d_dst_rgb_sorted; f.w2 = c->color_weight; }
  for (int i = 0; i < 9; ++i) f.M[i] = c->feat_M[i];
  const float x = c->normal_weight * c->src_nrm0[0], y = c->normal_weight * c->src_nrm0[1], z = c->normal_weight * c->src_nrm0[2];
  f.nw = std::sqrt(x * x + (y * y + z * z));
  return f;
}
static int ensure_feature_arrays(cilhip_ctx* c) {
  if (c->feature_kind == 0) return CILHIP_OK;
  if (!c->d_dst_rgb || !c->d_src_rgb) return fail(c, CILHIP_ERR_INVALID, "colour features: cilhip_set_color_features first");
  if (!c->dst_rgb_sorted_ok) {
    if (!c->d_dst_rgb_sorted) CK(c, hipMalloc(&c->d_dst_rgb_sorted, (c->grid.n ? c->grid.n : 1) * sizeof(float4)));
    launch_gather_by_w(c->grid.pts, c->d_dst_rgb, c->grid.n, c->d_dst_rgb_sorted, c->stream);
    c->dst_rgb_sorted_ok = true;
  }
  return CILHIP_OK;
}

static IterArgs make_iter_args(cilhip_ctx* c, float max_sq) {
  IterArgs a{};
  a.grid = c->grid;
  a.src = c->d_src_sorted;
  a.src_nrm = (c->d_src_nrm && c->symmetric) ? c->d_src_nrm_sorted : nullptr;
  a.feat = feat_spec_of(c);
  a.ns = c->ns;
  a.max_sq = max_sq;
  for (int i = 0; i < 3; ++i) a.dst_mean[i] = c->dst_mean[i];
  for (int i = 0; i < 9; ++i) a.tile_axes[i] = c->tile_axes[i];
  a.state = c->d_state;
  a.nn_pos = c->d_nn_pos;
  a.nn_d2 = c->d_nn_d2;
  a.partials = c->d_partials;
  a.defer_mask = c->d_defer_mask;
  a.tile_partials = c->d_partials;
  a.defer_flag = c->d_defer_flag;
  a.unproven_cnt = c->d_unproven;
  a.store_matches = 1;
  a.skip_if_inner_done = 0;
  a.tie = tie_dev_of(c);
  return a;
}

static int launch_search(cilhip_ctx* c, const IterArgs& a, int lanes = -1 ) {
  if (lanes < 0) lanes = c->group_lanes > 0 ? c->group_lanes : 0;
  if (feat6(c)) {
    if (c->feature_kind != 1 && (!c->has_normals || !c->d_src_nrm)) return fail(c, CILHIP_ERR_INVALID, "point+normal features need target and source normals");
    if (c->feature_kind == 1 && (!a.feat.src || !a.feat.dst)) return fail(c, CILHIP_ERR_INVALID, "colour features: cilhip_set_color_features first");
    if (c->feature_kind == 2 && (!a.feat.src2 || !a.feat.dst2)) return fail(c, CILHIP_ERR_INVALID, "point+normal+colour features: cilhip_set_color_features first");
    if (c->index_offset) return fail(c, CILHIP_ERR_UNSUPPORTED, "feature adaptors are not available on target shards");
    if (use_tiled(c)) launch_search_tiled_feat6(a, c->d_tiles, c->d_tile_center, c->d_tile_box, c->ntiles, c->stream);
    else launch_search_feat6(a, c->stream);
    return CILHIP_OK;
  }
  if (use_tiled(c)) launch_search_tiled(a, IM_NONE, c->d_tiles, c->d_tile_center, c->d_tile_box, c->ntiles, c->stream);
  else if (lanes) launch_search_group(a, lanes, c->stream);
  else launch_iter(a, IM_NONE, true, true, iter_num_blocks(c->ns), c->stream);
  return CILHIP_OK;
}

static int ensure_src_grid(cilhip_ctx* c) {
  if (!c->has_src_grid && c->ns) {
    GridBuildResult r{};
    double mean[3];
    const float* attr = c->feature_kind == 1 ? c->d_src_rgb : c->d_src_nrm;
    const hipError_t eg = build_grid(c->d_src_xyz, attr, c->ns, c->stream, &r, mean, 1.0);
    if (eg != hipSuccess) { c->err = std::string("build_grid (source): ") + hipGetErrorString(eg); return CILHIP_ERR_HIP; }
    c->src_grid = r.grid; c->has_src_grid = true;
  }
  if (c->has_src_grid && c->feature_kind == 2 && c->d_src_rgb && !c->d_src_rgb_grid) {
    CK(c, hipMalloc(&c->d_src_rgb_grid, (c->ns ? c->ns : 1) * sizeof(float4)));
    launch_gather_by_w(c->src_grid.pts, c->d_src_rgb, c->ns, c->d_src_rgb_grid, c->stream);
  }
  return CILHIP_OK;
}

static int ensure_reverse_buffers(cilhip_ctx* c) {
  const int rc = ensure_src_grid(c);
  if (rc) return rc;
  if (!c->d_rev_pos) {
    CK(c, hipMalloc(&c->d_rev_pos, (c->grid.n ? c->grid.n : 1) * sizeof(uint32_t)));
    CK(c, hipMalloc(&c->d_rev_d2, (c->grid.n ? c->grid.n : 1) * sizeof(float)));
  }
  if (!c->d_src_safe2 && c->has_src_grid && c->reverse_warm) {
    CK(c, hipMalloc(&c->d_src_safe2, (c->ns ? c->ns : 1) * sizeof(float)));
    launch_self_nn(c->src_grid, c->d_src_safe2, c->stream);
  }
  if (!c->d_src_inv) {
    CK(c, hipMalloc(&c->d_src_inv, (c->ns ? c->ns : 1) * sizeof(uint32_t)));
    launch_inv_perm(c->d_src_sorted, c->ns, c->d_src_inv, c->stream);
  }
  if (!c->d_grid_to_sorted && c->has_src_grid) {
    CK(c, hipMalloc(&c->d_grid_to_sorted, (c->ns ? c->ns : 1) * sizeof(uint32_t)));
    launch_grid_to_sorted(c->src_grid.pts, c->ns, c->d_src_inv, c->d_grid_to_sorted, c->stream);
  }
  return CILHIP_OK;
}

static int run_pair_search(cilhip_ctx* c, const IterArgs& a, float max_sq, const float T_host[16]) {
  if (!c->d_state_id) {
    CK(c, hipMalloc(&c->d_state_id, sizeof(IcpState)));
    const float zero[3] = {0, 0, 0};
    launch_init_state(c->d_state_id, kIdentity, zero, c->stream);
  }
  if (c->search_dir == 2 && c->ns && c->grid.n) {
    const int src_rc = launch_search(c, a);
    if (src_rc) return src_rc;
  }
  { const int grc = ensure_src_grid(c); if (grc) return grc; }
  FeatSpec rf = a.feat;
  rf.src = c->has_src_grid ? c->src_grid.nrm : nullptr;
  if (rf.dst2) rf.src2 = c->d_src_rgb_grid;
  if (feat6(c) && (!rf.src || !rf.dst || (rf.dst2 && !rf.src2))) return fail(c, CILHIP_ERR_INVALID, "feature search: both clouds' feature vectors are needed");
  if (!feat6(c)) { rf.w = 0.0f; rf.enabled = 0; }
  if (c->rev_tie_aware && tie_mode_on(c)) { const int trc = build_rev_tie_tables(c, T_host); if (trc) return trc; }
  const TieDev rt = tie_dev_rev(c);
  const hipError_t e = find_pairs(rf, c->grid, c->src_grid, c->d_src_xyz, (c->d_src_nrm && c->symmetric) ? c->d_src_nrm : nullptr, c->d_src_sorted, c->ns, c->d_state,
                                  c->d_state_id, T_host, max_sq, c->search_dir, c->reciprocal, c->inlier_fraction, c->one_to_one, c->d_nn_pos, c->d_nn_d2,
                                  c->pairs, c->stream, &rt);
  if (e != hipSuccess) { c->err = std::string("find_pairs: ") + hipGetErrorString(e); return CILHIP_ERR_HIP; }
  return CILHIP_OK;
}

// ... 1678 lines not shown
```

### cilantro_amd/csrc/grid_build.hip

```cpp
#include <hip/hip_runtime.h>

#include <cstring>

#include <rocprim/device/device_radix_sort.hpp>
#include <rocprim/device/device_scan.hpp>
#include <rocprim/iterator/reverse_iterator.hpp>

#include <algorithm>
#include <cmath>
#include <vector>

#include "internal.hpp"

namespace cilhip {

#define HIP_TRY(x) do { hipError_t e_ = (x); if (e_ != hipSuccess) return e_; } while (0)

constexpr int RB = 1024;

__global__ __launch_bounds__(256) void k_bbox_sum(const float* __restrict__ xyz, uint32_t n, float* bmin, float* bmax, double* bsum) {
  float mn[3] = {INFINITY, INFINITY, INFINITY}, mx[3] = {-INFINITY, -INFINITY, -INFINITY};
  double sm[3] = {0, 0, 0};
  const uint32_t per = (n + gridDim.x - 1) / gridDim.x;
  const uint32_t beg = blockIdx.x * per, end = min(beg + per, n);
// ... 209 lines not shown
    set_dims(g, lo, hi, cell);
    ncells = (size_t)g.nx * g.ny * g.nz;
    if (cs) { (void)hipFree(cs); cs = nullptr; }
    HIP_TRY(hipMalloc(&cs, (ncells + 1) * sizeof(uint32_t)));
    hipLaunchKernelGGL(k_cell_keys, dim3(grid_blocks(n)), dim3(256), 0, s, d_xyz, n, g, k_in, v_in);
    HIP_TRY(sort_pairs(k_in, k_out, v_in, v_out, n, bits_for((uint32_t)ncells), s));
    HIP_TRY(cell_start_table(k_out, n, (uint32_t)ncells, cs, s));
    HIP_TRY(hipMemsetAsync(d_occ, 0, sizeof(double), s));
    hipLaunchKernelGGL(k_occupancy, dim3(grid_blocks((uint32_t)ncells)), dim3(256), 0, s, cs, (uint32_t)ncells, d_occ);
    HIP_TRY(hipMemcpyAsync(&occ, d_occ, sizeof(double), hipMemcpyDeviceToHost, s));
    HIP_TRY(hipStreamSynchronize(s));
    occ /= (double)n;
    const double RF = refined_factor >= 1.0 ? refined_factor : 1.0;
    if (occ <= 3.0 * TARGET * (attempt == 0 ? 1.0 : RF)) break;
    const double shrink = std::min(0.85, std::max(0.3, std::pow(2.0 * TARGET * RF / occ, 1.0 / 2.5)));
    const double new_cell = (double)g.cell * shrink;
    GridDev probe = g;
    set_dims(probe, lo, hi, new_cell);
    if (probe.cell >= g.cell * 0.97f) break;
    cell = new_cell;
  }
  float4 *pts = nullptr, *nrm = nullptr;
  HIP_TRY(hipMalloc(&pts, (size_t)n * sizeof(float4)));
  if (d_nrm) HIP_TRY(hipMalloc(&nrm, (size_t)n * sizeof(float4)));
  hipLaunchKernelGGL(k_gather, dim3(grid_blocks(n)), dim3(256), 0, s, d_xyz, d_nrm, v_out, n, pts, nrm);
  HIP_TRY(hipStreamSynchronize(s));
  (void)hipFree(k_in); (void)hipFree(k_out); (void)hipFree(v_in); (void)hipFree(v_out); (void)hipFree(d_occ);
  g.pts = pts; g.nrm = nrm; g.cell_start = cs;
  out->grid = g; out->avg_occupancy = occ; out->n_cells = ncells;
  return hipSuccess;
}

void free_grid(GridDev& g) {
  if (g.pts) (void)hipFree((void*)g.pts);
  if (g.nrm) (void)hipFree((void*)g.nrm);
  if (g.pn) (void)hipFree((void*)g.pn);
  if (g.cell_start) (void)hipFree((void*)g.cell_start);
  g.pts = nullptr; g.nrm = nullptr; g.pn = nullptr; g.cell_start = nullptr;
}

__device__ __forceinline__ uint32_t cube_key_of(const GridDev& g, float x, float y, float z) {
  int cx = (int)floorf(fminf(fmaxf((x - g.ox) * g.inv_cell, -1.0f), 1.0e9f));
  int cy = (int)floorf(fminf(fmaxf((y - g.oy) * g.inv_cell, -1.0f), 1.0e9f));
  int cz = (int)floorf(fminf(fmaxf((z - g.oz) * g.inv_cell, -1.0f), 1.0e9f));
  cx = min(max(cx - GRID_PAD, 0), g.nx - 1 - GRID_PAD); cy = min(max(cy - GRID_PAD, 0), g.ny - 1 - GRID_PAD); cz = min(max(cz - GRID_PAD, 0), g.nz - 1 - GRID_PAD);
  constexpr uint32_t C = CUBE_EDGE;
  const uint32_t cnx = (uint32_t)(g.nx - 1 - GRID_PAD) / C + 1, cny = (uint32_t)(g.ny - 1 - GRID_PAD) / C + 1;
  const uint32_t bx = (uint32_t)cx / C, by = (uint32_t)cy / C, bz = (uint32_t)cz / C;
  const uint32_t cube = (bz * cny + by) * cnx + bx;
  const uint32_t local = (((uint32_t)cz - bz * C) * C + ((uint32_t)cy - by * C)) * C + ((uint32_t)cx - bx * C);
  return cube * (C * C * C) + local;
}

__global__ void k_cube_keys_tf(const float* __restrict__ xyz, uint32_t n, GridDev g, Tf T, uint32_t* keys, uint32_t* vals) {
  for (uint32_t i = blockIdx.x * blockDim.x + threadIdx.x; i < n; i += gridDim.x * blockDim.x) {
    float qx, qy, qz;
    transform_point(T.m, xyz[3 * (size_t)i], xyz[3 * (size_t)i + 1], xyz[3 * (size_t)i + 2], qx, qy, qz);
    keys[i] = cube_key_of(g, qx, qy, qz);
    vals[i] = i;
  }
}

__global__ void k_shift_keys(const uint32_t* __restrict__ in, uint32_t n, uint32_t* out) {
  for (uint32_t i = blockIdx.x * blockDim.x + threadIdx.x; i < n; i += gridDim.x * blockDim.x) out[i] = in[i] / (uint32_t)(CUBE_EDGE * CUBE_EDGE * CUBE_EDGE);
}

__global__ void k_tile_counts(const uint32_t* __restrict__ cube_start, uint32_t ncubes, uint32_t* counts) {
  for (uint32_t c = blockIdx.x * blockDim.x + threadIdx.x; c < ncubes; c += gridDim.x * blockDim.x)
    counts[c] = (cube_start[c + 1] - cube_start[c] + (TILE_QUERIES - 1)) / TILE_QUERIES;
}

__global__ void k_emit_tiles(const uint32_t* __restrict__ cube_start, const uint32_t* __restrict__ tile_off, uint32_t ncubes, GridDev g, Tf Tinv,
                             uint2* tiles, float4* tile_center) {
  constexpr uint32_t C = CUBE_EDGE;
  const uint32_t cnx = (uint32_t)(g.nx - 1 - GRID_PAD) / C + 1, cny = (uint32_t)(g.ny - 1 - GRID_PAD) / C + 1;
  for (uint32_t c = blockIdx.x * blockDim.x + threadIdx.x; c < ncubes; c += gridDim.x * blockDim.x) {
    const uint32_t b = cube_start[c], e = cube_start[c + 1];
    if (b == e) continue;
    const uint32_t bx = c % cnx, by = (c / cnx) % cny, bz = c / (cnx * cny);
    const float hx = g.ox + ((float)(bx * C) + (float)GRID_PAD + 0.5f * (float)C) * g.cell, hy = g.oy + ((float)(by * C) + (float)GRID_PAD + 0.5f * (float)C) * g.cell,
                hz = g.oz + ((float)(bz * C) + (float)GRID_PAD + 0.5f * (float)C) * g.cell;
    const float* m = Tinv.m;
    const float4 ctr = make_float4(m[0] * hx + m[4] * hy + m[8] * hz + m[12], m[1] * hx + m[5] * hy + m[9] * hz + m[13],
                                   m[2] * hx + m[6] * hy + m[10] * hz + m[14], 0.0f);
    uint32_t t = tile_off[c];
    for (uint32_t q = b; q < e; q += TILE_QUERIES) { tiles[t] = make_uint2(q, min(q + TILE_QUERIES, e)); tile_center[t] = ctr; ++t; }
  }
}

hipError_t sort_source(const float* d_xyz, uint32_t n, const GridDev& g, const float T[16], float4* d_out, hipStream_t s,
                       uint2** d_tiles_out, float4** d_tile_center_out, float tile_axes_out[9], uint32_t* ntiles_out, SortWorkspace* ws) {
  *d_tiles_out = nullptr; *d_tile_center_out = nullptr; *ntiles_out = 0;
  Tf tinv;
  {
    const double a00 = T[0], a01 = T[4], a02 = T[8], a10 = T[1], a11 = T[5], a12 = T[9], a20 = T[2], a21 = T[6], a22 = T[10];
    const double det = a00 * (a11 * a22 - a12 * a21) - a01 * (a10 * a22 - a12 * a20) + a02 * (a10 * a21 - a11 * a20);
    const double id = (det != 0.0 && std::isfinite(det)) ? 1.0 / det : 0.0;
    const double i00 = (a11 * a22 - a12 * a21) * id, i01 = (a02 * a21 - a01 * a22) * id, i02 = (a01 * a12 - a02 * a11) * id;
    const double i10 = (a12 * a20 - a10 * a22) * id, i11 = (a00 * a22 - a02 * a20) * id, i12 = (a02 * a10 - a00 * a12) * id;
    const double i20 = (a10 * a21 - a11 * a20) * id, i21 = (a01 * a20 - a00 * a21) * id, i22 = (a00 * a11 - a01 * a10) * id;
    const double t0 = T[12], t1 = T[13], t2 = T[14];
    const double inv[16] = {i00, i10, i20, 0, i01, i11, i21, 0, i02, i12, i22, 0,
                            -(i00 * t0 + i01 * t1 + i02 * t2), -(i10 * t0 + i11 * t1 + i12 * t2), -(i20 * t0 + i21 * t1 + i22 * t2), 1};
    for (int i = 0; i < 16; ++i) tinv.m[i] = (float)inv[i];
    const double h = 0.5 * (double)CUBE_EDGE * (double)g.cell;
    const double li[9] = {i00, i01, i02, i10, i11, i12, i20, i21, i22};
    for (int i = 0; i < 9; ++i) tile_axes_out[i] = (float)(h * li[i]);
  }
  if (n == 0) return hipSuccess;
  constexpr uint32_t CE = CUBE_EDGE;
  const uint32_t cnx = (uint32_t)(g.nx - 1 - GRID_PAD) / CE + 1, cny = (uint32_t)(g.ny - 1 - GRID_PAD) / CE + 1, cnz = (uint32_t)(g.nz - 1 - GRID_PAD) / CE + 1;
  const uint32_t ncubes = cnx * cny * cnz;
  const unsigned bits = std::min(32u, bits_for(ncubes * CE * CE * CE));
  uint32_t* nul = nullptr;
  size_t sort_tmp = 0, scan_tmp = 0;
  HIP_TRY(rocprim::radix_sort_pairs(nullptr, sort_tmp, nul, nul, nul, nul, (size_t)n, 0u, bits, s));
  HIP_TRY(rocprim::exclusive_scan(nullptr, scan_tmp, nul, nul, 0u, (size_t)ncubes + 1, rocprim::plus<uint32_t>(), s));
  auto up = [](size_t b) { return (b + 255) & ~(size_t)255; };
  const size_t arr = up((size_t)n * 4), carr = up(((size_t)ncubes + 1) * 4);
  const size_t need = 4 * arr + 3 * carr + up(sort_tmp ? sort_tmp : 16) + up(scan_tmp ? scan_tmp : 16);
  SortWorkspace local;
  SortWorkspace* w = ws ? ws : &local;
  hipError_t e = hipSuccess;
  if (w->scratch_bytes < need) {
    if (w->scratch) (void)hipFree(w->scratch);
    w->scratch = nullptr; w->scratch_bytes = 0;
    if ((e = hipMalloc(&w->scratch, need)) != hipSuccess) return e;
    w->scratch_bytes = need;
  }
  char* base = static_cast<char*>(w->scratch);
  uint32_t *k_in = reinterpret_cast<uint32_t*>(base), *k_out = reinterpret_cast<uint32_t*>(base + arr), *v_in = reinterpret_cast<uint32_t*>(base + 2 * arr),
           *v_out = reinterpret_cast<uint32_t*>(base + 3 * arr);
  uint32_t *cube_start = reinterpret_cast<uint32_t*>(base + 4 * arr), *tcount = reinterpret_cast<uint32_t*>(base + 4 * arr + carr),
           *toff = reinterpret_cast<uint32_t*>(base + 4 * arr + 2 * carr);
  void* tmp_sort = base + 4 * arr + 3 * carr;
  void* tmp_scan = base + 4 * arr + 3 * carr + up(sort_tmp ? sort_tmp : 16);
  Tf tf;
  for (int i = 0; i < 16; ++i) tf.m[i] = T[i];
  uint2* tiles = nullptr;
  float4* centers = nullptr;
  do {
    hipLaunchKernelGGL(k_cube_keys_tf, dim3(grid_blocks(n)), dim3(256), 0, s, d_xyz, n, g, tf, k_in, v_in);
    if ((e = rocprim::radix_sort_pairs(tmp_sort, sort_tmp, k_in, k_out, v_in, v_out, (size_t)n, 0u, bits, s)) != hipSuccess) break;
    hipLaunchKernelGGL(k_gather, dim3(grid_blocks(n)), dim3(256), 0, s, d_xyz, (const float*)nullptr, v_out, n, d_out, (float4*)nullptr);
    hipLaunchKernelGGL(k_shift_keys, dim3(grid_blocks(n)), dim3(256), 0, s, k_out, n, k_in);
    hipLaunchKernelGGL(k_cell_start, dim3(grid_blocks(n + 1)), dim3(256), 0, s, k_in, n, ncubes, cube_start);
    if ((e = hipMemsetAsync(tcount, 0, ((size_t)ncubes + 1) * 4, s)) != hipSuccess) break;
    hipLaunchKernelGGL(k_tile_counts, dim3(grid_blocks(ncubes)), dim3(256), 0, s, cube_start, ncubes, tcount);
    if ((e = rocprim::exclusive_scan(tmp_scan, scan_tmp, tcount, toff, 0u, (size_t)ncubes + 1, rocprim::plus<uint32_t>(), s)) != hipSuccess) break;
    uint32_t ntiles = 0;
    if ((e = hipMemcpyAsync(&ntiles, toff + ncubes, 4, hipMemcpyDeviceToHost, s)) != hipSuccess) break;
    if ((e = hipStreamSynchronize(s)) != hipSuccess) break;
    if (ws) {
      if (ws->tile_cap < ntiles + 1) {
        if (ws->tiles) (void)hipFree(ws->tiles);
        if (ws->centers) (void)hipFree(ws->centers);
        ws->tiles = nullptr; ws->centers = nullptr; ws->tile_cap = 0;
        const uint32_t cap = ntiles + 1 + ntiles / 8;
        if ((e = hipMalloc(&ws->tiles, (size_t)cap * sizeof(uint2))) != hipSuccess) break;
        if ((e = hipMalloc(&ws->centers, (size_t)cap * sizeof(float4))) != hipSuccess) break;
        ws->tile_cap = cap;
      }
      tiles = ws->tiles; centers = ws->centers;
    } else {
      if ((e = hipMalloc(&tiles, ((size_t)ntiles + 1) * sizeof(uint2))) != hipSuccess) break;
      if ((e = hipMalloc(&centers, ((size_t)ntiles + 1) * sizeof(float4))) != hipSuccess) break;
    }
    hipLaunchKernelGGL(k_emit_tiles, dim3(grid_blocks(ncubes)), dim3(256), 0, s, cube_start, toff, ncubes, g, tinv, tiles, centers);
    e = ws ? hipGetLastError() : hipStreamSynchronize(s);
    *d_tiles_out = tiles; *d_tile_center_out = centers; *ntiles_out = ntiles;
  } while (0);
  if (!ws) {
    (void)hipStreamSynchronize(s);
    if (local.scratch) (void)hipFree(local.scratch);
    if (e != hipSuccess) {
      if (tiles) (void)hipFree(tiles);
      if (centers) (void)hipFree(centers);
    }
  }
  if (e != hipSuccess) { *d_tiles_out = nullptr; *d_tile_center_out = nullptr; *ntiles_out = 0; }
  return e;
}

void free_sort_workspace(SortWorkspace& ws) {
  if (ws.scratch) (void)hipFree(ws.scratch);
  if (ws.tiles) (void)hipFree(ws.tiles);
  if (ws.centers) (void)hipFree(ws.centers);
  ws = SortWorkspace();
}

}
```

### cilantro_amd/csrc/internal.hpp

```cpp
#pragma once

#include <hip/hip_runtime.h>
#include <stdint.h>

#include <string>
#include <thread>

#include "solve.hpp"

struct cilhip_ctx;

namespace cilhip {

constexpr uint32_t NONE_U32 = 0xFFFFFFFFu;
#ifndef CILHIP_CUBE_EDGE
#define CILHIP_CUBE_EDGE 12
#endif
constexpr int CUBE_EDGE = CILHIP_CUBE_EDGE;
constexpr int GRID_PAD = 2;
#ifndef CILHIP_TILE_THREADS
#define CILHIP_TILE_THREADS 1024
#endif
#ifndef CILHIP_TILE_WAVES_PER_SIMD
#define CILHIP_TILE_WAVES_PER_SIMD 8
// ... 43 lines not shown
  unsigned int listed;
  int violation_iter;
  float violation_delta;
  unsigned long long violation_ncorr;
  float violation_T[16];
  float Tprev[16];
  float motion_acc, motion_eps, motion_step;
  float motion_pred;
  unsigned int tie_counters[4];
};

enum IterMetric { IM_NONE = 0, IM_KABSCH = 1, IM_PLANE = 2, IM_POINT = 3, IM_BOTH = 4,
                  IM_AFF0 = 5,
                  IM_AFF1 = 6,
                  IM_AFF2 = 7,
                  IM_AFFC = 8, IM_AFFP = 9 };
inline bool im_affine_fused(int m) { return m == IM_AFFC || m == IM_AFFP; }
constexpr int AFF_ROW = 128;
constexpr int AFF_SUMS = 94;

enum { CW_UNITY = 0, CW_IDENTITY = 1, CW_RBF = 2 };
struct CorrWeights {
  int enabled;
  int point_kind, plane_kind;
  float point_coeff, plane_coeff;
  float w_p2p, w_p2pl;
  const float* point_table;
  const float* plane_table;
};

struct F3 { float x, y, z; };

struct TieDev {
  const uint2* leaf_slot;
  const uint4* nodes;
  unsigned int* counters;
  int mode;
};

struct FeatSpec {
  const float4* src;
  const float4* dst;
  float w;
  int enabled;
  int mode;
  float M[9];
  float nw;
  const float4* src2;
  const float4* dst2;
  float w2;
};

struct IterArgs {
  GridDev grid;
  const float4* src;
  const float4* src_nrm;
  uint32_t ns;
  float max_sq;
  float dst_mean[3];
  float tile_axes[9];
  const IcpState* state;
  uint32_t* nn_pos;
  float* nn_d2;
  double* partials;
  unsigned long long* defer_mask;
  double* tile_partials;
  uint32_t* defer_flag;
  uint32_t* unproven_cnt;
  int store_matches;
  int skip_if_inner_done;
  int no_centering;
  FeatSpec feat;
  CorrWeights cw;
  const uint32_t* warm_pos;
  float warm_far_sq;
  float warm_extra;
  float4* warm_rec;
  F3* warm_rec_n;
  F3* warm_src3;
  const float* safe2;
  float* nn_lb;
  int lb_valid;
  TieDev tie;
};

struct BoxArgs {
  const float4* tile_center;
  int* tile_box;
  uint32_t ntiles;
  uint32_t* defer_flag;
  float ox, oy, oz, inv_cell;
  int nx, ny, nz;
  float tile_axes[9];
  int trim;
};

struct FeedbackSlot {
  unsigned int unproven;
  unsigned int listed;
  float delta;
  float prev_delta;
  float step;
  float pad;
  unsigned long long commit;
};
struct Feedback {
  FeedbackSlot slot[4];
  unsigned long long latest;
};

struct SolveArgs {
  Feedback* feedback;
  unsigned int run_tag;
  IcpState* state;
  const double* partials;
  int nblocks;
  const double* reduced;
  int metric;
  float w_p2p, w_p2pl;
  int point_weighted;
  float conv_tol, opt_conv_tol;
  float dst_mean[3], src_mean[3];
  int gn_last_step;
  int gn_zero_steps;
  int has_normals;
  int affine_centered;
  uint32_t* unproven_cnt;
  int guard_axis;
  float guard_slack;
  float guard_center[3], guard_half[3];
  float guard_T[16];
  float src_center[3], src_half[3];
  uint4* trace;
};
constexpr int RUN_TRACE_CAP = 256;

#if defined(__HIPCC__)
__device__ __forceinline__ bool tie_before(const TieDev& tt, float qx, float qy, float qz, uint32_t pa, uint32_t pb) {
  const uint2 la = tt.leaf_slot[pa], lb = tt.leaf_slot[pb];
  if (la.x == lb.x) return la.y < lb.y;
  uint32_t na = la.x, nb = lb.x;
  uint4 A = tt.nodes[na], B = tt.nodes[nb];
  uint32_t a_second = 0;
  while ((A.y >> 3) > (B.y >> 3)) { a_second = A.y & 1u; na = A.x; A = tt.nodes[na]; }
  while ((B.y >> 3) > (A.y >> 3)) { nb = B.x; B = tt.nodes[nb]; }
  while (na != nb) { a_second = A.y & 1u; na = A.x; A = tt.nodes[na]; nb = B.x; B = tt.nodes[nb]; }
  const uint32_t feat = (A.y >> 1) & 3u;
  const float val = feat == 0u ? qx : (feat == 1u ? qy : qz);
  const float diff1 = __fsub_rn(val, __uint_as_float(A.z)), diff2 = __fsub_rn(val, __uint_as_float(A.w));
  const uint32_t first_is_second = __fadd_rn(diff1, diff2) < 0.0f ? 0u : 1u;
  return a_second == first_is_second;
}
__device__ __forceinline__ void source_feature(const FeatSpec& a, const float* T , const float4 sn, float& fx, float& fy, float& fz) {
  const float wx = __fmul_rn(a.w, sn.x), wy = __fmul_rn(a.w, sn.y), wz = __fmul_rn(a.w, sn.z);
  if (a.mode == 2) { fx = wx; fy = wy; fz = wz; return; }
  if (a.mode == 1) {
    const float* M = a.M;
    const float v0 = __fadd_rn(__fmul_rn(M[0], wx), __fadd_rn(__fmul_rn(M[1], wy), __fmul_rn(M[2], wz)));
    const float v1 = __fadd_rn(__fmul_rn(M[3], wx), __fadd_rn(__fmul_rn(M[4], wy), __fmul_rn(M[5], wz)));
    const float v2 = __fadd_rn(__fmul_rn(M[6], wx), __fadd_rn(__fmul_rn(M[7], wy), __fmul_rn(M[8], wz)));
    const float nrm = (float)sqrt((double)__fadd_rn(__fmul_rn(v0, v0), __fadd_rn(__fmul_rn(v1, v1), __fmul_rn(v2, v2))));
    if (!(nrm > 0.0f)) { fx = __fmul_rn(a.nw, v0); fy = __fmul_rn(a.nw, v1); fz = __fmul_rn(a.nw, v2); return; }
    fx = __fmul_rn(a.nw, (float)((double)v0 / (double)nrm));
    fy = __fmul_rn(a.nw, (float)((double)v1 / (double)nrm));
    fz = __fmul_rn(a.nw, (float)((double)v2 / (double)nrm));
    return;
  }
  fx = __fadd_rn(__fmul_rn(T[0], wx), __fadd_rn(__fmul_rn(T[4], wy), __fmul_rn(T[8], wz)));
  fy = __fadd_rn(__fmul_rn(T[1], wx), __fadd_rn(__fmul_rn(T[5], wy), __fmul_rn(T[9], wz)));
  fz = __fadd_rn(__fmul_rn(T[2], wx), __fadd_rn(__fmul_rn(T[6], wy), __fmul_rn(T[10], wz)));
}
__device__ __forceinline__ float d6_features(float ax, float ay, float az, float afx, float afy, float afz, float bx, float by, float bz, float bfx, float bfy,
                                             float bfz) {
  const float d0 = __fsub_rn(ax, bx), d1 = __fsub_rn(ay, by), d2 = __fsub_rn(az, bz);
  const float d3 = __fsub_rn(afx, bfx), d4 = __fsub_rn(afy, bfy), d5 = __fsub_rn(afz, bfz);
// ... 35 lines not shown
void launch_reduce_partials(const double* partials, int nblocks, double* stage, double* out, hipStream_t s);
void launch_reduce_stage1_groups(const double* partials, int nblocks, double* stage, int groups, hipStream_t s);
int launch_reduce_stage1(const double* partials, int nblocks, double* stage, hipStream_t s);
void launch_reduce_and_solve(const double* partials, int nblocks, double* stage, unsigned int* ticket, SolveArgs a, hipStream_t s);
constexpr int REDUCE_STAGE_DOUBLES = 128 * SUMS_MAX;
int affine_acc_blocks(uint32_t ns);
void launch_acc_affine(const IterArgs& a, int metric, int nblocks, hipStream_t s);
void launch_reduce_and_solve_affine(const double* partials, int nrows, double* stage , const SolveArgs& a, hipStream_t s);
void launch_init_state(IcpState* st, const float T0[16], const float src_mean[3], hipStream_t s, Feedback* fb = nullptr, unsigned int run_tag = 0,
                       const float* src_center = nullptr, const float* src_half = nullptr, unsigned int* tie_counters = nullptr );
void launch_scatter_nn(const float4* src_sorted, const float4* dst_sorted, const uint32_t* nn_pos,
                       const float* nn_d2, uint32_t ns, uint32_t* out_idx, float* out_d2,
                       hipStream_t s);
void launch_gather_by_w(const float4* src_sorted, const float* in_xyz, uint32_t ns, float4* out, hipStream_t s);
void launch_gather1_by_w(const float4* src_sorted, const float* in, uint32_t ns, float* out, hipStream_t s);
void launch_pack_keys(const float4* src_sorted, const float4* dst_sorted, const uint32_t* nn_pos, const float* nn_d2,
                      uint32_t ns, uint32_t index_offset, unsigned long long* keys, hipStream_t s);
void launch_keys_to_pos(const float4* src_sorted, const unsigned long long* keys, const uint32_t* inv_perm, uint32_t ns,
                        uint32_t index_offset, uint32_t n_local, uint32_t* nn_pos, float* nn_d2, hipStream_t s, unsigned int* tie_counter = nullptr);
void launch_order_keys(const float4* src_sorted, const IcpState* state, const unsigned long long* win, const uint32_t* nn_pos, const float* nn_d2,
                       uint32_t ns, const TieDev& tt, unsigned long long* own, unsigned long long* out, hipStream_t s);
void launch_select_ordered(const float4* src_sorted, const unsigned long long* own, const unsigned long long* reduced, const unsigned long long* win,
                           uint32_t ns, uint32_t* nn_pos, float* nn_d2, hipStream_t s);
void launch_inv_perm(const float4* dst_sorted, uint32_t n, uint32_t* inv, hipStream_t s);
void launch_count_found(const uint32_t* nn_pos, uint32_t ns, unsigned long long* out, hipStream_t s);
void launch_transform_original_host_T(const float* d_src_xyz, uint32_t ns, const float T[16], float* d_out, hipStream_t s);
struct TieNode {
  int32_t parent;
  uint32_t info;
  float divlow, divhigh;
};
extern int g_knn_tie_rule;
hipError_t tie_order_build_device(const float* d_xyz, const float4* d_sorted, uint32_t n, hipStream_t s, uint32_t* d_leaf_by_index, uint32_t* d_slot_by_index,
                                  uint4** d_nodes_out, size_t* n_nodes_out, int* max_depth_out);
hipError_t tie_order_build_device_features(int dim, const float4* d_sorted, const float4* att1, float w1, const float4* att2, float w2, uint32_t n, hipStream_t s,
                                           uint32_t* d_leaf_by_index, uint32_t* d_slot_by_index, uint4** d_nodes_out, size_t* n_nodes_out, int* max_depth_out);
void launch_tie_tables_by_position(const float4* dst_sorted, uint32_t n, const uint32_t* leaf_by_index, const uint32_t* slot_by_index, uint2* leaf_slot, hipStream_t s);
void launch_count_ties(const GridDev& g, const float4* src_sorted, uint32_t ns, const float T[16], float max_sq, unsigned long long* out, hipStream_t s);
void launch_fill_d2(const float4* src_sorted, const float4* dst_sorted, const uint32_t* nn_pos, const float T[16], uint32_t ns, float* nn_d2, hipStream_t s);
void launch_residuals(const IterArgs& a, int metric, float w_p2p, float w_p2pl, float* out, hipStream_t s);
int iter_num_blocks(uint32_t ns);
void launch_acc_reverse(const IterArgs& a, int metric, const float4* sgrid_pts, const uint32_t* rev_pos, uint32_t nd, int mode, const uint32_t* fwd_pos,
                        const uint32_t* src_inv, int nblocks, hipStream_t s);

void launch_filter_fraction(const float4* src_sorted, uint32_t* nn_pos, const float* nn_d2, uint32_t ns, double fraction,
                            unsigned long long* keys, void* state, hipStream_t s);
void launch_filter_one_to_one(const float4* src_sorted, uint32_t* nn_pos, const float* nn_d2, uint32_t ns,
                              unsigned long long* winner, uint32_t n_target, hipStream_t s);
size_t filter_state_bytes();
void launch_select_fraction(const float* d2, uint32_t n, double fraction, unsigned long long* keys, void* state, uint32_t* flags, hipStream_t s);

struct PairSet {
  uint32_t *first = nullptr, *second = nullptr;
  uint32_t *posd = nullptr, *poss = nullptr;
  float* d2 = nullptr;
  uint32_t *first2 = nullptr, *second2 = nullptr, *posd2 = nullptr, *poss2 = nullptr;
  float* d2b = nullptr;
  float4 *src_view = nullptr, *nrm_view = nullptr;
  size_t cap = 0;
  uint32_t count = 0;
  static constexpr int WS_COUNT = 15;
  void* ws[WS_COUNT] = {nullptr, nullptr, nullptr, nullptr, nullptr, nullptr, nullptr, nullptr, nullptr, nullptr, nullptr, nullptr, nullptr, nullptr, nullptr};
  size_t ws_cand = 0, ws_tmp_bytes = 0, ws_nd = 0, ws_ns = 0;
};
void free_pairs(PairSet& p);
struct RevFused { int metric; int mode; const uint32_t* fwd_pos; const uint32_t* src_inv; const uint32_t* grid_to_sorted; double* partials; float dst_mean[3]; };
void launch_grid_to_sorted(const float4* sgrid_pts, uint32_t ns, const uint32_t* src_inv, uint32_t* out , hipStream_t s);
int reverse_warm_blocks(uint32_t nd);
void launch_reverse_search_rigid(const GridDev& g, const GridDev& src_grid, const IcpState* state, float max_sq, uint32_t* rev_pos, float* rev_d2, hipStream_t s,
                                 const FeatSpec* feat = nullptr, const TieDev* rev_tie = nullptr, const float* warm_src_safe2 = nullptr, const RevFused* fused = nullptr);
hipError_t find_pairs(const FeatSpec& feat, const GridDev& g, const GridDev& src_grid , const float* d_src_xyz, const float* d_src_nrm,
                      const float4* src_sorted, uint32_t ns, const IcpState* state, const IcpState* id_state, const float T_host[16], float max_sq,
                      int direction, bool reciprocal, double inlier_fraction, bool one_to_one, const uint32_t* fwd_pos, const float* fwd_d2,
                      PairSet& out, hipStream_t s, const TieDev* rev_tie = nullptr);

struct GridBuildResult {
  GridDev grid;
  double avg_occupancy;
  size_t n_cells;
};
hipError_t build_grid(const float* d_xyz, const float* d_nrm, uint32_t n, hipStream_t s,
                      GridBuildResult* out, double mean_out[3], double target_occupancy, double refined_factor = 1.0);
void free_grid(GridDev& g);
struct SortWorkspace {
  void* scratch = nullptr; size_t scratch_bytes = 0;
  uint2* tiles = nullptr; float4* centers = nullptr; uint32_t tile_cap = 0;
};
hipError_t sort_source(const float* d_xyz, uint32_t n, const GridDev& g, const float T[16], float4* d_out,
                       hipStream_t s, uint2** d_tiles_out, float4** d_tile_center_out, float tile_axes_out[9], uint32_t* ntiles_out,
                       SortWorkspace* ws = nullptr);
void free_sort_workspace(SortWorkspace& ws);
hipError_t mean3_device(const float* d_xyz, uint32_t n, hipStream_t s, double mean_out[3], float* lo_out = nullptr, float* hi_out = nullptr);

hipStream_t ctx_stream(const ::cilhip_ctx* c);
double ctx_wait_us(const ::cilhip_ctx* c);
constexpr float kIdentity16[16] = {1, 0, 0, 0, 0, 1, 0, 0, 0, 0, 1, 0, 0, 0, 0, 1};
inline void cpu_relax(unsigned spins) {
#if defined(__x86_64__) || defined(__i386__)
  __builtin_ia32_pause();
#endif
  if ((spins & 255u) == 255u) std::this_thread::yield();
}
}
```

### cilantro_amd/csrc/kernels.hip

```cpp
#include "search_device.hpp"

namespace cilhip {

void set_launch_events(hipEvent_t start, hipEvent_t stop) { g_ev_start = start; g_ev_stop = stop; }

constexpr int TILE_MAXE = CILHIP_TILE_MAXE;
constexpr int TILE_QPT = TILE_QUERIES / TILE_THREADS;
constexpr int TILE_WAVES = TILE_THREADS / 64;
constexpr uint32_t DEFER_MARK = 0xFFFFFFFEu;
static_assert(FUSED_WAVE_BYTES * TILE_WAVES <= TILE_BYTES, "the accumulation scratch reuses the tile's point buffer");
static_assert(TILE_CAP + 8 < 65536, "LDS slots are packed into 16 bits");
static_assert(TILE_MAXE <= 65536 && TILE_MAXROWS <= 32767, "OctQuery packs a table index and a row into 16 bits each");
static_assert(TILE_MAXROWS <= 64 * 8, "the row scan holds at most 8 rows per lane of one wave");

typedef float f32x2 __attribute__((ext_vector_type(2)));

__device__ __forceinline__ uint32_t umed3(uint32_t a, uint32_t b, uint32_t c) {
  uint32_t r;
  asm("v_med3_u32 %0, %1, %2, %3" : "=v"(r) : "v"(a), "v"(b), "v"(c));
  return r;
}

struct Run4 { f32x2 x0, y0, z0, x1, y1, z1; };

// ... 289 lines not shown
      bl = x.bl; e1 = x.e1; second = x.e2; tie = x.tie;
    }
    if (!(e1 < max_sq)) { second = fminf(second, e1); bl = NONE_U32; e1 = max_sq; tie = false; }
  }
  second = fminf(second, max_sq);
  best.key = ((unsigned long long)__float_as_uint(e1) << 32);
  uint32_t pos = NONE_U32;
  if (bl != NONE_U32) {
    if (bl >= t.rowbase[brow] && bl < t.rowbase[brow + 1]) pos = bl + t.rowdelta[brow];
    else pos = lds_to_global(bl, t.rowbase, t.rowdelta, t.rows);
  }
  best.pos = pos;
  const float ux = qx_ - (g.ox + (float)cx * g.cell), uy = qy_ - (g.oy + (float)cy * g.cell), uz = qz_ - (g.oz + (float)cz * g.cell);
  float bd = INFINITY;
  if (cx - 1 > 0) bd = fminf(bd, ux);
  if (cx + 2 < g.nx) bd = fminf(bd, g.cell - ux);
  if (cy - 1 > 0) bd = fminf(bd, uy);
  if (cy + 2 < g.ny) bd = fminf(bd, g.cell - uy);
  if (cz - 1 > 0) bd = fminf(bd, uz);
  if (cz + 2 < g.nz) bd = fminf(bd, g.cell - uz);
  if (second_out) *second_out = second;
  if (tie) { if (bound_out) *bound_out = 0.0f; return false; }
  if (bd == INFINITY) { if (bound_out) *bound_out = INFINITY; return true; }
  bd = fmaxf(bd, 0.0f) + g.cell - 2.0f * g.margin;
  if (bound_out) *bound_out = bd;
  return bd > 0.0f && e1 < bd * bd * KSHRINK;
}

#ifdef CILHIP_EXP_PHASE_CLOCKS
__device__ unsigned long long g_phase_clk[8];
#define PHASE_CLK(k) do { if (threadIdx.x == 0) { const unsigned long long now_ = wall_clock64(); atomicAdd(&g_phase_clk[k], now_ - tprev_); tprev_ = now_; } } while (0)
void debug_dump_warm_clocks();
void debug_dump_phase_clocks() {
  debug_dump_warm_clocks();
  unsigned long long h[8];
  if (hipMemcpyFromSymbol(h, HIP_SYMBOL(g_phase_clk), sizeof h) != hipSuccess) return;
  unsigned long long tot = 0;
  for (int k = 0; k < 8; ++k) tot += h[k];
  fprintf(stderr, "[phase clocks, 100 MHz ticks summed over blocks, thread 0] table=%llu scan+prep=%llu stage=%llu search(+3b, masks)=%llu tail loads+z=%llu mfma+D=%llu row=%llu total=%llu\n",
          h[0], h[1], h[2], h[3], h[4], h[5], h[6], tot);
  memset(h, 0, sizeof h);
  (void)hipMemcpyToSymbol(HIP_SYMBOL(g_phase_clk), h, sizeof h);
}
#else
#define PHASE_CLK(k)
#endif

__device__ __forceinline__ void compute_tile_box(const float* T, const BoxArgs& g, uint32_t t) {
  const bool trim = g.trim != 0;
  const float4 c4 = g.tile_center[t];
  float ccx, ccy, ccz;
  transform_point(T, c4.x, c4.y, c4.z, ccx, ccy, ccz);
  float ext[3];
#pragma unroll
  for (int i = 0; i < 3; ++i) {
    float e = 0.0f;
#pragma unroll
    for (int k = 0; k < 3; ++k)
      e += fabsf(T[i] * g.tile_axes[k] + T[i + 4] * g.tile_axes[3 + k] + T[i + 8] * g.tile_axes[6 + k]);
    ext[i] = e;
  }
  const float SHR = 1.0e-3f, BIG = 1.0e9f;
  const float HALF_SLACK = 0.01f;
  int lo[3], hi[3];
  const float cc3[3] = {ccx, ccy, ccz}, o3[3] = {g.ox, g.oy, g.oz};
  const int n3[3] = {g.nx, g.ny, g.nz};
#pragma unroll
  for (int i = 0; i < 3; ++i) {
    const float a0 = fminf(fmaxf((cc3[i] - ext[i] - o3[i]) * g.inv_cell + SHR, -BIG), BIG);
    const float a1 = fminf(fmaxf((cc3[i] + ext[i] - o3[i]) * g.inv_cell - SHR, -BIG), BIG);
    int b0 = (int)floorf(a0), b1 = (int)floorf(a1);
    bool halo0 = !trim || (a0 - (float)b0) < 0.5f + HALF_SLACK, halo1 = !trim || (a1 - (float)b1) > 0.5f - HALF_SLACK;
    if (b0 <= GRID_PAD) { b0 = min(b0, GRID_PAD - 1); halo0 = true; }
    if (b1 >= n3[i] - 1 - GRID_PAD) { b1 = max(b1, n3[i] - GRID_PAD); halo1 = true; }
    lo[i] = b0 - (halo0 ? 1 : 0) + 1;
    hi[i] = b1 + (halo1 ? 1 : 0) - 1;
  }
  const int bx0 = lo[0], bx1 = hi[0], by0 = lo[1], by1 = hi[1], bz0 = lo[2], bz1 = hi[2];
  const int W1 = (min(bx1 + 1, g.nx - 1) - max(bx0 - 1, 0) + 1) + 1, RY = min(by1 + 1, g.ny - 1) - max(by0 - 1, 0) + 1;
  const uint32_t inv_w1 = W1 > 0 ? ((1u << 20) + (uint32_t)W1 - 1u) / (uint32_t)W1 : 0u;
  const uint32_t inv_ry = RY > 0 ? (65536u + (uint32_t)RY - 1u) / (uint32_t)RY : 0u;
  int* b = g.tile_box + 8 * (size_t)t;
  b[0] = bx0; b[1] = bx1; b[2] = by0; b[3] = by1; b[4] = bz0; b[5] = bz1; b[6] = (int)inv_w1; b[7] = (int)inv_ry;
}


__global__ void k_tile_boxes(BoxArgs g, const IcpState* __restrict__ st) {
  if (st->done) return;
  const uint32_t t = blockIdx.x * blockDim.x + threadIdx.x;
  if (t == 0) *g.defer_flag = 0u;
  if (t >= g.ntiles) return;
  float T[16];
#pragma unroll
  for (int k = 0; k < 16; ++k) T[k] = st->T[k];
  compute_tile_box(T, g, t);
}

BoxArgs make_box_args(const IterArgs& a, const float4* tile_center, int* tile_box, uint32_t ntiles, bool trim) {
  BoxArgs b{};
  b.tile_center = tile_center; b.tile_box = tile_box; b.ntiles = ntiles; b.defer_flag = a.defer_flag;
  b.ox = a.grid.ox; b.oy = a.grid.oy; b.oz = a.grid.oz; b.inv_cell = a.grid.inv_cell;
  b.nx = a.grid.nx; b.ny = a.grid.ny; b.nz = a.grid.nz;
  for (int i = 0; i < 9; ++i) b.tile_axes[i] = a.tile_axes[i];
  b.trim = trim ? 1 : 0;
  return b;
}

template <int ACC>
__device__ __forceinline__ void defer_whole_tile(const IterArgs& a, uint32_t vb) {
  if ((threadIdx.x & 63u) == 0) {
#pragma unroll
    for (int u = 0; u < TILE_QPT; ++u) a.defer_mask[(size_t)vb * (2 * TILE_WAVES) + u * TILE_WAVES + (threadIdx.x >> 6)] = ~0ull;
    if (threadIdx.x == 0) { if (__hip_atomic_load(a.defer_flag, __ATOMIC_RELAXED, __HIP_MEMORY_SCOPE_AGENT) == 0u) __hip_atomic_store(a.defer_flag, 1u, __ATOMIC_RELAXED, __HIP_MEMORY_SCOPE_AGENT); atomicAdd(a.unproven_cnt + (vb & 63u), (uint32_t)TILE_QUERIES); atomicAdd(a.unproven_cnt + 64u + (vb & 63u), (uint32_t)TILE_QUERIES); }
  }
  if (ACC != IM_NONE && threadIdx.x < SUMS_MAX) a.tile_partials[(size_t)vb * SUMS_MAX + threadIdx.x] = 0.0;
}

template <int ACC, bool FEAT6 = false, bool LB = false>
__global__ __launch_bounds__(TILE_THREADS, CILHIP_TILE_WAVES_PER_SIMD) void k_search_tiled(IterArgs a, const uint2* __restrict__ tiles,
                                                                  const int* __restrict__ tile_box, uint32_t ntiles) {
  static_assert(!(LB && FEAT6), "margin keys are a property of the 3-D point search");
  const IcpState* __restrict__ st = a.state;
  if (st->done) return;
  const uint32_t per = (ntiles + 7u) >> 3;
  const uint32_t vb = (blockIdx.x & 7u) * per + (blockIdx.x >> 3);
  if ((blockIdx.x >> 3) >= per || vb >= ntiles) return;

  __shared__ __attribute__((aligned(16))) unsigned char raw[TILE_BYTES];
  __shared__ uint32_t lcs[TILE_MAXE];
  __shared__ uint32_t rowbase[TILE_MAXROWS + 1];
  __shared__ uint32_t rowdelta[TILE_MAXROWS];
  __shared__ uint32_t queue_count;
  __shared__ float tform_lds[19];
  __shared__ uint32_t small_count;
  __shared__ int geom_lds[8];
  float* const lp = reinterpret_cast<float*>(raw);
  if (threadIdx.x == 0) { queue_count = 0; small_count = 0; }
  if (threadIdx.x < 16) tform_lds[threadIdx.x] = st->T[threadIdx.x];
  if (LB && threadIdx.x == 16) { tform_lds[16] = st->motion_acc; tform_lds[17] = st->motion_eps; tform_lds[18] = st->motion_pred; }
#ifdef CILHIP_EXP_PHASE_CLOCKS
  unsigned long long tprev_ = wall_clock64();
#endif

  const GridDev& g = a.grid;
  const uint2 tile = tiles[vb];
  float T[16];
#pragma unroll
  for (int k = 0; k < 16; ++k) T[k] = st->T[k];
  const float smt[3] = {st->smt[0], st->smt[1], st->smt[2]};
  const MotionRef mref = {LB ? st->motion_acc : 0.0f, LB ? st->motion_eps : 0.0f};
  const float mstep = LB ? st->motion_pred : 0.0f;

  float4 s4[TILE_QPT];
#pragma unroll
  for (int u = 0; u < TILE_QPT; ++u) {
    const uint32_t i = tile.x + u * TILE_THREADS + threadIdx.x;
    s4[u] = i < tile.y ? a.src[i] : make_float4(0.f, 0.f, 0.f, 0.f);
  }

  const int* tb = tile_box + 8 * (size_t)vb;
  const int bx0 = tb[0], bx1 = tb[1], by0 = tb[2], by1 = tb[3], bz0 = tb[4], bz1 = tb[5];
  const int lox = max(bx0 - 1, 0), loy = max(by0 - 1, 0), loz = max(bz0 - 1, 0);
  const int hix = min(bx1 + 1, g.nx - 1), hiy = min(by1 + 1, g.ny - 1), hiz = min(bz1 + 1, g.nz - 1);
  const int RX = hix - lox + 1, RY = hiy - loy + 1, RZ = hiz - loz + 1;
  int rows = RY * RZ;
  const int W1 = RX + 1, E = rows * W1;
  const int fx0 = max(bx0, 1), fx1 = min(bx1, g.nx - 2), fy0 = max(by0, 1), fy1 = min(by1, g.ny - 2), fz0 = max(bz0, 1), fz1 = min(bz1, g.nz - 2);
  bool ok = (fx0 <= fx1) & (fy0 <= fy1) & (fz0 <= fz1) & (RY <= TILE_MAXSPAN) & (RZ <= TILE_MAXSPAN) & (E <= TILE_MAXE);
  if (!ok) {
    defer_whole_tile<ACC>(a, vb);
    return;
  }

  if (threadIdx.x == 0) { geom_lds[0] = lox; geom_lds[1] = loy; geom_lds[2] = loz; geom_lds[3] = RY; geom_lds[4] = W1; geom_lds[5] = rows; }

  const __amdgpu_buffer_rsrc_t rs_cs = __builtin_amdgcn_make_buffer_rsrc(
      (void*)g.cell_start, 0, ((uint32_t)g.nx * (uint32_t)g.ny * (uint32_t)g.nz + 1u) * 4u, 0x00020000);
  {
    const uint32_t inv_w1 = (uint32_t)tb[6], inv_ry = (uint32_t)tb[7];
    constexpr int TRIPS = (TILE_MAXE + TILE_THREADS - 1) / TILE_THREADS;
    const uint32_t rowstride = (uint32_t)g.nx, slab = (uint32_t)g.ny * (uint32_t)g.nx;
    const uint32_t gbase = ((uint32_t)loz * (uint32_t)g.ny + (uint32_t)loy) * (uint32_t)g.nx + (uint32_t)lox;
    uint32_t v[TRIPS];
#pragma unroll
    for (int k = 0; k < TRIPS; ++k) {
      if (k * TILE_THREADS < E) {
        const uint32_t e = (uint32_t)k * TILE_THREADS + threadIdx.x;
        const uint32_t r = __umul24(e, inv_w1) >> 20;
        const uint32_t x = e - __umul24(r, (uint32_t)W1);
        const uint32_t zr = __umul24(r, inv_ry) >> 16;
        const uint32_t gi = gbase + __umul24(zr, slab) + __umul24(r - __umul24(zr, (uint32_t)RY), rowstride) + x;
        v[k] = __builtin_amdgcn_raw_buffer_load_b32(rs_cs, e < (uint32_t)E ? gi * 4u : 0xFFFFFFFFu, 0, 0);
      }
    }
#pragma unroll
    for (int k = 0; k < TRIPS; ++k) {
      if (k * TILE_THREADS < E) {
        const uint32_t e = (uint32_t)k * TILE_THREADS + threadIdx.x;
        if (e < (uint32_t)E) lcs[e] = v[k];
      }
    }
  }
  __syncthreads();
  PHASE_CLK(0);

  if (threadIdx.x < 64) {
    const int K = (rows + 63) >> 6;
    const int r0 = (int)threadIdx.x * K;
    uint32_t len[8], fst[8], tot = 0;
#pragma unroll
    for (int k = 0; k < 8; ++k) {
      const int r = r0 + k;
      const bool v = (k < K) & (r < rows);
      fst[k] = v ? lcs[r * W1] : 0u;
      len[k] = v ? lcs[r * W1 + RX] - fst[k] : 0u;
      tot += len[k];
    }
    uint32_t incl = tot;
#pragma unroll
    for (int off = 1; off < 64; off <<= 1) {
      const uint32_t tt = __shfl_up(incl, off, 64);
      if ((int)threadIdx.x >= off) incl += tt;
    }
    uint32_t run = incl - tot;
#pragma unroll
    for (int k = 0; k < 8; ++k) {
      const int r = r0 + k;
      if ((k < K) & (r < rows)) {
        rowbase[r] = run;
        rowdelta[r] = fst[k] - run;
        run += len[k];
      }
    }
    if (threadIdx.x == 63) rowbase[rows] = incl;
  }

  OctQuery oq[TILE_QPT];
  uint32_t flags = 0;
#pragma unroll
  for (int u = 0; u < TILE_QPT; ++u) {
    const uint32_t i = tile.x + u * TILE_THREADS + threadIdx.x;
    float qx, qy, qz;
    transform_point(T, s4[u].x, s4[u].y, s4[u].z, qx, qy, qz);
    const float BIG = 1.0e9f;
    const int cx = (int)floorf(fminf(fmaxf((qx - g.ox) * g.inv_cell, -BIG), BIG));
    const int cy = (int)floorf(fminf(fmaxf((qy - g.oy) * g.inv_cell, -BIG), BIG));
    const int cz = (int)floorf(fminf(fmaxf((qz - g.oz) * g.inv_cell, -BIG), BIG));
    const bool active = i < tile.y;
    const bool fast = active & octant_prepare(g, qx, qy, qz, cx, cy, cz, lox, loy, loz, hix, hiy, hiz, RY, W1, oq[u]);
    flags |= (active ? (1u << u) : 0u) | (fast ? (1u << (8 + u)) : 0u);
  }
  __syncthreads();
  PHASE_CLK(1);
  uint32_t P = rowbase[rows];
  if (P > (uint32_t)TILE_CAP) {
    int rz = RZ;
    while (rz > 3 && rowbase[rz * RY] > (uint32_t)TILE_CAP) --rz;
    if (rowbase[rz * RY] > (uint32_t)TILE_CAP) {
      defer_whole_tile<ACC>(a, vb);
      return;
    }
    rows = rz * RY;
    P = rowbase[rows];
    const int fz1n = loz + rz - 2;
#pragma unroll
    for (int u = 0; u < TILE_QPT; ++u)
      if ((int)floorf((oq[u].qz - g.oz) * g.inv_cell) > fz1n) flags &= ~(1u << (8 + u));
    if (threadIdx.x == 0) geom_lds[5] = rows;
  }
  {
    typedef uint32_t u32x4 __attribute__((ext_vector_type(4)));
    const __amdgpu_buffer_rsrc_t rs_pts = __builtin_amdgcn_make_buffer_rsrc((void*)g.pts, 0, g.n * 16u, 0x00020000);
    const uint32_t o0 = threadIdx.x & 15;
    const int grp = threadIdx.x >> 4;
    constexpr int GR = TILE_THREADS / 16;
#ifndef CILHIP_STAGE_ROWS
#define CILHIP_STAGE_ROWS 4
#endif
    constexpr int STAGE_ROWS = CILHIP_STAGE_ROWS;
    for (int rb = 0; rb < rows; rb += STAGE_ROWS * GR) {
#pragma unroll
      for (int half = 0; half < 2; ++half) {
        u32x4 v[STAGE_ROWS];
        uint32_t dst[STAGE_ROWS];
#pragma unroll
        for (int m = 0; m < STAGE_ROWS; ++m) {
          const int r = rb + grp + GR * m;
          const bool rv = r < rows;
          const uint32_t f = rv ? rowbase[r] : 0u, l = rv ? rowbase[r + 1] - f : 0u, d = rv ? rowdelta[r] : 0u;
          const uint32_t o = o0 + 16u * (uint32_t)half;
          const bool has = o < l;
          dst[m] = has ? f + o : NONE_U32;
          v[m] = __builtin_amdgcn_raw_buffer_load_b128(rs_pts, has ? (f + o + d) * 16u : 0xFFFFFFFFu, 0, 0);
        }
#pragma unroll
        for (int m = 0; m < STAGE_ROWS; ++m)
          if (dst[m] != NONE_U32) {
            float* const w = lp + lds_slot_x(dst[m]);
            w[0] = __uint_as_float(v[m].x); w[2] = __uint_as_float(v[m].y); w[4] = __uint_as_float(v[m].z);
          }
      }
    }
    for (int r = grp; r < rows; r += GR) {
      const uint32_t f = rowbase[r], l = rowbase[r + 1] - f, d = rowdelta[r];
      for (uint32_t o = o0 + 32u; o < l; o += 16) { const float4 q = g.pts[f + o + d]; float* const w = lp + lds_slot_x(f + o); w[0] = q.x; w[2] = q.y; w[4] = q.z; }
    }
    if (threadIdx.x < 30) lp[lds_slot_x(P + threadIdx.x / 3u) + 2u * (threadIdx.x % 3u)] = 1.0e30f;
  }
  __syncthreads();
  PHASE_CLK(2);
  TileLds tl{lp, (uint32_t)reinterpret_cast<uintptr_t>(raw), (P + 1u) & ~1u, lcs, rowbase, rowdelta, lox, loy, loz, RY, W1, rows};
  uint32_t mpos[TILE_QPT];
  uint32_t mbl = 0;
  uint32_t mkeys = 0;
  uint32_t f6_pos[TILE_QPT];
  float f6_second[TILE_QPT];
#pragma unroll
  for (int u = 0; u < TILE_QPT; ++u) {
    const bool active = (flags >> u) & 1u, fast = (flags >> (8 + u)) & 1u;
    const uint32_t i = tile.x + u * TILE_THREADS + threadIdx.x;
    NN best;
    best.key = ((unsigned long long)__float_as_uint(a.max_sq) << 32);
    best.pos = NONE_U32;
    uint32_t bl = NONE_U32;
    bool defer = false, unproven = false, pending = false;
    float mkey = 0.0f;
    uint32_t mq = 0;
    if (active) {
      if (fast && FEAT6) {
        (void)octant_search(g, tl, oq[u], a.max_sq, best, bl, &f6_second[u]);
        f6_pos[u] = best.pos;
        mbl |= (bl & 0xFFFFu) << (16 * u);
        pending = true;
      } else if (fast) {
        float second = INFINITY, gapb = 0.0f;
        unproven = !octant_search(g, tl, oq[u], a.max_sq, best, bl, &second, &gapb);
        if (LB && ACC == IM_NONE) mkey = margin_key(best.pos != NONE_U32, second, gapb, mref);
        if (LB && ACC != IM_NONE) mq = margin_q15(best.pos != NONE_U32, second, gapb, mref, g.inv_cell);
        if (LB) {
          const bool small = unproven ? (ACC != IM_NONE) : margin_is_small(best.pos != NONE_U32, second, gapb, __uint_as_float((uint32_t)(best.key >> 32)), a.max_sq, mstep);
          const unsigned long long ms = __ballot(small);
          if (ms != 0ull && (threadIdx.x & 63u) == 0) atomicAdd(&small_count, (uint32_t)__popcll(ms));
        }
      } else {
        const float gx = axis_gap(oq[u].qx, g.ox, g.ox + (float)g.nx * g.cell, g.margin);
        const float gy = axis_gap(oq[u].qy, g.oy, g.oy + (float)g.ny * g.cell, g.margin);
        const float gz = axis_gap(oq[u].qz, g.oz, g.oz + (float)g.nz * g.cell, g.margin);
        defer = (gx * gx + gy * gy + gz * gz) * KSHRINK < a.max_sq;
        const float ggap = __fsqrt_rn((gx * gx + gy * gy + gz * gz) * KSHRINK) * 0.999999f;
        if (LB && ACC == IM_NONE) mkey = margin_key(false, INFINITY, ggap, mref);
        if (LB && ACC != IM_NONE) mq = margin_q15(false, INFINITY, ggap, mref, g.inv_cell);
      }
    }
    if (ACC != IM_NONE || FEAT6) {
      const unsigned long long mu = __ballot(unproven);
      if (mu != 0ull && (threadIdx.x & 63u) == 0) atomicAdd(&queue_count, (uint32_t)__popcll(mu));
      if (unproven) { defer = true; unproven = false; }
    }
    const unsigned long long m = (ACC == IM_NONE && !FEAT6) ? __ballot(unproven) : 0ull;
    if (m) {
      const int lane = (int)(threadIdx.x & 63u), leader = __ffsll((long long)m) - 1;
      uint32_t base = 0;
      if (lane == leader) base = atomicAdd(&queue_count, (uint32_t)__popcll(m));
      base = __shfl(base, leader, 64);
      const uint32_t slot = base + (uint32_t)__popcll(m & ((1ull << lane) - 1ull));
      const uint32_t Pq = (uint32_t)__builtin_amdgcn_readfirstlane((int)rowbase[rows]);
      uint16_t* const queue = reinterpret_cast<uint16_t*>(raw + ((Pq + 12u) >> 1) * 24u);
      const uint32_t queue_cap = min((uint32_t)TILE_QUERIES, ((uint32_t)TILE_CAP - Pq) * 6u);
      if (unproven) {
        if (slot < queue_cap) {
          queue[slot] = (uint16_t)(u * TILE_THREADS + threadIdx.x);
        }
      }
    }
    if (active && !unproven && !defer && !pending && a.store_matches) {
      a.nn_pos[i] = best.pos;
      if (a.nn_d2) a.nn_d2[i] = __uint_as_float((uint32_t)(best.key >> 32));
    }
    if (LB && ACC == IM_NONE && active && !unproven && !defer) a.nn_lb[i] = mkey;
    if (LB && ACC != IM_NONE) mkeys |= ((active && !defer) ? mq : 0u) << (16 * u);
    mpos[u] = (unproven | defer) ? NONE_U32 : best.pos;
    if (ACC != IM_NONE) mbl |= (bl & 0xFFFFu) << (16 * u);
    flags |= (unproven ? (1u << (16 + u)) : 0u) | (defer ? (1u << (24 + u)) : 0u) | (pending ? (1u << (20 + u)) : 0u);
  }
  if (FEAT6) {
    float4 np[TILE_QPT], cp[TILE_QPT], rr[TILE_QPT];
#pragma unroll
    for (int u = 0; u < TILE_QPT; ++u) {
      np[u] = cp[u] = rr[u] = make_float4(0.f, 0.f, 0.f, 0.f);
      if (((flags >> (20 + u)) & 1u) && f6_pos[u] != NONE_U32) {
        np[u] = target_features(a)[f6_pos[u]];
        if (a.feat.dst2 != nullptr) cp[u] = a.feat.dst2[f6_pos[u]];
// ... 789 lines not shown
```

### cilantro_amd/icp.py

```python
import ctypes as C
from enum import Enum

import numpy as np

from . import capi


class CorrespondenceSearchDirection(Enum):
    FIRST_TO_SECOND = 0
    SECOND_TO_FIRST = 1
    BOTH = 2


def _is_torch(x):
    return type(x).__module__.startswith("torch")


def _as_cloud(x):
    if x is None:
        return None, 0, capi.MEM_HOST, None
    if _is_torch(x):
        import torch

        t = x
# ... 209 lines not shown

    def icp_iterate_ranked(self, iterations):
        self._ck(self._L.cilhip_icp_iterate_ranked(self._h, int(iterations)))

    def last_host_enqueue_time(self):
        v = C.c_double(0)
        self._ck(self._L.cilhip_get_last_host_enqueue_time(self._h, C.byref(v)))
        return v.value

    def get_option(self, key):
        v = C.c_double(0)
        self._ck(self._L.cilhip_get_option(self._h, key.encode(), C.byref(v)))
        return v.value

    def last_allreduce_timing(self):
        a = C.c_double(0); n = C.c_int(0)
        self._ck(self._L.cilhip_get_last_allreduce_timing(self._h, C.byref(a), C.byref(n)))
        return a.value, n.value

    def set_shard_info(self, target_index_offset, dst_mean=None, src_mean=None):
        dm = np.ascontiguousarray(dst_mean, np.float32) if dst_mean is not None else None
        sm = np.ascontiguousarray(src_mean, np.float32) if src_mean is not None else None
        self._ck(self._L.cilhip_set_shard_info(self._h, int(target_index_offset), dm.ctypes.data if dm is not None else None,
                                               sm.ctypes.data if sm is not None else None))

    def icp_partial_keys(self, keys_dev_ptr):
        self._ck(self._L.cilhip_icp_partial_keys(self._h, C.c_void_p(keys_dev_ptr)))

    def icp_sums_from_keys(self, keys_dev_ptr, sums_dev_ptr):
        self._ck(self._L.cilhip_icp_sums_from_keys(self._h, C.c_void_p(keys_dev_ptr), C.c_void_p(sums_dev_ptr)))

    def icp_order_keys(self, win_keys_dev_ptr, order_keys_dev_ptr):
        self._ck(self._L.cilhip_icp_order_keys(self._h, C.c_void_p(win_keys_dev_ptr), C.c_void_p(order_keys_dev_ptr)))

    def icp_sums_from_ordered_keys(self, win_keys_dev_ptr, order_keys_dev_ptr, sums_dev_ptr):
        self._ck(self._L.cilhip_icp_sums_from_ordered_keys(self._h, C.c_void_p(win_keys_dev_ptr), C.c_void_p(order_keys_dev_ptr), C.c_void_p(sums_dev_ptr)))

    def set_slab_guard(self, axis, slack=0.0, center=None, half_extent=None, T_part=None):
        if axis is None or axis < 0:
            self._ck(self._L.cilhip_set_slab_guard(self._h, -1, C.c_float(0.0), None, None, None))
            return
        c = np.ascontiguousarray(center, np.float32); h = np.ascontiguousarray(half_extent, np.float32); t = _T_to_abi(T_part)
        self._ck(self._L.cilhip_set_slab_guard(self._h, int(axis), C.c_float(slack), c.ctypes.data, h.ctypes.data, t.ctypes.data))

    def slab_violation(self):
        v = C.c_int(0)
        self._ck(self._L.cilhip_get_slab_violation(self._h, C.byref(v)))
        return bool(v.value)

    def slab_violation_state(self):
        v = C.c_int(0); res = capi.IcpResult()
        self._ck(self._L.cilhip_get_slab_violation_state(self._h, C.byref(v), C.byref(res)))
        return bool(v.value), res

    def icp_state(self):
        res = capi.IcpResult()
        self._ck(self._L.cilhip_icp_state(self._h, C.byref(res)))
        return res

    def compute_residuals(self, metric, w_p2p, w_p2pl, T):
        out = np.zeros(max(self.n_source, 1), np.float32)
        t = _T_to_abi(T)
        self._ck(self._L.cilhip_compute_residuals(self._h, metric, w_p2p, w_p2pl, t.ctypes.data, out.ctypes.data, capi.MEM_HOST))
        return out[: self.n_source]

    def prepare_source(self, T=None, force=False):
        ms = C.c_double(0)
        t = None if T is None else _T_to_abi(T)
        self._ck(self._L.cilhip_prepare_source(self._h, None if t is None else t.ctypes.data, 1 if force else 0, C.byref(ms)))
        return ms.value

    def grid_info(self):
        gi = capi.GridInfo()
        self._ck(self._L.cilhip_get_grid_info(self._h, C.byref(gi)))
        return gi

    def enable_kernel_timing(self, on=True):
        self._ck(self._L.cilhip_enable_kernel_timing(self._h, 1 if on else 0))

    def debug_counters(self):
        out = (C.c_uint32 * 2)()
        self._ck(self._L.cilhip_debug_counters(self._h, out))
        return int(out[0]), int(out[1])

    def set_option(self, key, value):
        self._ck(self._L.cilhip_set_option(self._h, key.encode(), float(value)))

    def set_pair_weight_callback(self, fn):
        if fn is None:
            self._weight_cb = None
            self._ck(self._L.cilhip_set_pair_weight_callback(self._h, capi.PAIR_WEIGHT_FN(), None))
            return

        def tramp(_user, i1, i2, val, n, wq, wl):
            try:
                if getattr(self, "_weight_exc", None) is not None:
                    return
                n = int(n)
                a1 = np.ctypeslib.as_array(i1, shape=(n,)); a2 = np.ctypeslib.as_array(i2, shape=(n,)); v = np.ctypeslib.as_array(val, shape=(n,))
                q, l = fn(a1, a2, v)
                np.ctypeslib.as_array(wq, shape=(n,))[:] = np.asarray(q, np.float32)
                np.ctypeslib.as_array(wl, shape=(n,))[:] = np.asarray(l, np.float32)
            except BaseException as e:
                self._weight_exc = e

        self._weight_cb = capi.PAIR_WEIGHT_FN(tramp)
        self._ck(self._L.cilhip_set_pair_weight_callback(self._h, self._weight_cb, None))

    def last_run_forms(self):
        a = C.c_int(0); b = C.c_int(0)
        self._ck(self._L.cilhip_get_last_run_forms(self._h, C.byref(a), C.byref(b)))
        return a.value, b.value

    def last_form_timing(self):
        out = {}
        for f in range(5):
            ms = C.c_double(0); n = C.c_int(0)
            self._ck(self._L.cilhip_get_last_form_timing(self._h, f, C.byref(ms), C.byref(n)))
            out[f] = (ms.value, n.value)
        return out

    def last_run_trace(self, cap=256):
        n = C.c_int(0)
        un = (C.c_uint * cap)(); li = (C.c_uint * cap)(); st = (C.c_float * cap)(); de = (C.c_float * cap)(); fo = (C.c_int * cap)()
        self._ck(self._L.cilhip_get_last_run_trace(self._h, cap, C.byref(n), un, li, st, de, fo))
        return [{"form": fo[i], "unproven": un[i], "listed": li[i], "step": st[i], "delta": de[i]} for i in range(n.value)]

    def last_iteration_timing(self, cap=4096):
        n = C.c_int(0)
        it = np.zeros(cap, np.uint32); ms = np.zeros(cap, np.float32)
        self._ck(self._L.cilhip_get_last_iteration_timing(self._h, cap, C.byref(n), it.ctypes.data, ms.ctypes.data))
        k = min(n.value, cap)
        return [(int(it[i]), float(ms[i])) for i in range(k)]

    def last_warm_iterations(self):
        a = C.c_int(0)
        self._ck(self._L.cilhip_get_last_warm_iterations(self._h, C.byref(a)))
        return a.value

    def last_matches_origin(self):
        a = C.c_int(0)
        self._ck(self._L.cilhip_get_last_matches_origin(self._h, C.byref(a)))
        return a.value

    def matches_transform(self):
        T = np.zeros(16, np.float32)
        self._ck(self._L.cilhip_get_matches_transform(self._h, T.ctypes.data))
        return _T_from_abi(T)

    def last_timing2(self):
        a = C.c_double(0); b = C.c_double(0)
        self._ck(self._L.cilhip_get_last_timing2(self._h, C.byref(a), C.byref(b)))
        return a.value, b.value

    def last_timing(self):
        a = C.c_double(0); b = C.c_double(0); n = C.c_int(0)
        self._ck(self._L.cilhip_get_last_timing(self._h, C.byref(a), C.byref(b), C.byref(n)))
        return a.value, b.value, n.value


class CorrespondenceSearchHIP:

    def __init__(self, ctx):
        self._ctx = ctx
        self.search_dir_ = CorrespondenceSearchDirection.SECOND_TO_FIRST
        self.max_distance_ = np.float32(0.01 * 0.01)
# ... 413 lines not shown
```

### include/cilantro_hip/c_api.h

```cpp
#ifndef CILANTRO_HIP_C_API_H
#define CILANTRO_HIP_C_API_H

#include <stddef.h>
#include <stdint.h>

#ifdef __cplusplus
extern "C" {
#endif

typedef struct cilhip_ctx cilhip_ctx;

typedef enum {
  CILHIP_OK = 0,
  CILHIP_ERR_INVALID = -1,
  CILHIP_ERR_HIP = -2,
  CILHIP_ERR_UNSUPPORTED = -3,
  CILHIP_ERR_NO_DEVICE = -4
} cilhip_status;

enum { CILHIP_MEM_HOST = 0, CILHIP_MEM_DEVICE = 1 };

enum {
  CILHIP_METRIC_POINT_TO_POINT = 0,
  CILHIP_METRIC_COMBINED = 1
// ... 125 lines not shown
int cilhip_transform_ransac3f(int device, const float* dst_xyz, const float* src_xyz, size_t n, int mem, const uint32_t* samples, uint64_t seed,
                              float max_residual, size_t target_inliers, size_t max_iter, int re_estimate, cilhip_transform_model* out,
                              float* residuals_out, uint32_t* inliers_out);
int cilhip_transform_score3f(int device, const float* dst_xyz, const float* src_xyz, size_t n, int mem, const float* transforms, size_t m,
                             float max_residual, uint32_t* counts_out);
int cilhip_transform_fit3f(int device, const float* dst_xyz, const float* src_xyz, size_t n, int mem, float T_out[16]);

int cilhip_knn_set_tie_rule(int rule);
int cilhip_knn3f(int device, const float* ref_xyz, size_t n_ref, const float* query_xyz, size_t n_query, int mem, size_t k,
                 float max_sq_dist, uint32_t* idx_out, float* d2_out, uint32_t* counts_out);
int cilhip_radius_search3f(int device, const float* ref_xyz, size_t n_ref, const float* query_xyz, size_t n_query, int mem,
                           float radius_sq, uint64_t* offsets_out, uint32_t* idx_out, float* d2_out, size_t capacity,
                           size_t* total_out_or_null);
int cilhip_normals_knn3f(int device, const float* xyz, size_t n, int mem, size_t k, float max_sq_dist, const float* view_point,
                         float* normals_out, float* curvature_out);
int cilhip_normals_radius3f(int device, const float* xyz, size_t n, int mem, float radius_sq, const float* view_point,
                            float* normals_out, float* curvature_out);

typedef struct {
  int nx, ny, nz;
  float cell;
  float origin[3];
  size_t n_cells;
  double avg_occupancy;
  double build_ms;
} cilhip_grid_info;
int cilhip_get_grid_info(cilhip_ctx* ctx, cilhip_grid_info* out);
int cilhip_get_tie_count(cilhip_ctx* ctx, const float T[16], float max_sq_dist, size_t* n_ties);
int cilhip_get_tie_rule_stats(cilhip_ctx* ctx, size_t* tied_queries, size_t* repointed);
typedef struct cilhip_tie_order_info { int loaded; int builds; double build_ms; size_t pending; } cilhip_tie_order_info;
int cilhip_get_tie_order_info(cilhip_ctx* ctx, cilhip_tie_order_info* out);
int cilhip_build_tie_order(cilhip_ctx* ctx);
typedef struct cilhip_tie_order cilhip_tie_order;
int cilhip_tie_order_create(const float* xyz, size_t n, cilhip_tie_order** out);
void cilhip_tie_order_destroy(cilhip_tie_order* order);
int cilhip_tie_order_tables(const cilhip_tie_order* order, uint32_t* leaf_by_index, uint32_t* slot_by_index, void* nodes_out, size_t nodes_cap,
                            size_t* n_nodes, int* max_depth);
int cilhip_load_tie_order(cilhip_ctx* ctx, const cilhip_tie_order* order, const uint32_t* global_index);

int cilhip_estimate_combined_two_sets(cilhip_ctx* ctx_point, cilhip_ctx* ctx_plane, float w_p2p, float w_p2pl, size_t max_iter, float conv_tol,
                                      float dT[16], int* converged);
int cilhip_icp_run_two_sets(cilhip_ctx* ctx_point, float max_sq_point, cilhip_ctx* ctx_plane, float max_sq_plane, const cilhip_icp_params* p,
                            const float* T0, cilhip_icp_result* out);

typedef struct cilhip_multi cilhip_multi;
int cilhip_multi_create(cilhip_multi** out, const int* devices, int ndev);
void cilhip_multi_destroy(cilhip_multi* m);
const char* cilhip_multi_last_error(const cilhip_multi* m);
cilhip_ctx* cilhip_multi_context(cilhip_multi* m, int rank);
int cilhip_multi_set_clouds(cilhip_multi* m, const float* dst_xyz, const float* dst_nrm_or_null, size_t n_dst, const float* src_xyz, size_t n_src,
                            float max_sq_dist, int partition, const float* T_part_or_null);
int cilhip_multi_icp_run(cilhip_multi* m, const cilhip_icp_params* p, const float* T0, int check_every, cilhip_icp_result* out);
int cilhip_multi_last_host_time(const cilhip_multi* m, double* us_per_iteration_per_shard);
int cilhip_multi_repartitions(const cilhip_multi* m);
int cilhip_multi_set_slab_slack(cilhip_multi* m, float slack);
int cilhip_multi_shard_sizes(const cilhip_multi* m, int rank, size_t* n_target, size_t* n_source);

int cilhip_rank_comm_unique_id(unsigned char id_out[128]);
int cilhip_rank_comm_prepare(cilhip_ctx* ctx);
int cilhip_rank_comm_init(cilhip_ctx* ctx, const unsigned char id[128], int nranks, int rank);
int cilhip_rank_comm_destroy(cilhip_ctx* ctx);
int cilhip_icp_iterate_ranked(cilhip_ctx* ctx, int iterations);
int cilhip_get_last_allreduce_timing(cilhip_ctx* ctx, double* total_ms, int* timed);
int cilhip_get_last_host_enqueue_time(cilhip_ctx* ctx, double* us_per_iteration);

int cilhip_get_last_run_forms(cilhip_ctx* ctx, int* one_pass_iterations, int* two_pass_iterations);
int cilhip_get_last_warm_iterations(cilhip_ctx* ctx, int* warm_iterations);
int cilhip_get_last_run_trace(cilhip_ctx* ctx, int cap, int* n, unsigned int* unproven, unsigned int* listed, float* step, float* delta, int* form);
int cilhip_get_last_form_timing(cilhip_ctx* ctx, int form, double* kernel_ms, int* launches);
int cilhip_get_last_iteration_timing(cilhip_ctx* ctx, int cap, int* n, unsigned int* iteration, float* kernel_ms);

int cilhip_get_last_timing(cilhip_ctx* ctx, double* loop_ms, double* search_kernel_ms,
                           int* search_kernel_launches);
int cilhip_enable_kernel_timing(cilhip_ctx* ctx, int on);
int cilhip_set_option(cilhip_ctx* ctx, const char* key, double value);
typedef enum cilhip_option {
  CILHIP_OPT_FUSED = 0, CILHIP_OPT_INLIER_FRACTION, CILHIP_OPT_ONE_TO_ONE, CILHIP_OPT_TILED, CILHIP_OPT_WARM_START, CILHIP_OPT_WARM_FORECAST,
  CILHIP_OPT_FUSED_EPILOGUE, CILHIP_OPT_GROUP_SEARCH, CILHIP_OPT_TIE_RULE, CILHIP_OPT_WARM_EXTRA_FRACTION, CILHIP_OPT_PAIR_RECORDS,
  CILHIP_OPT_TILE_RECORDS, CILHIP_OPT_WARM_ENTER_FRACTION, CILHIP_OPT_POINT_WEIGHT_EVALUATOR, CILHIP_OPT_PLANE_WEIGHT_EVALUATOR,
  CILHIP_OPT_POINT_WEIGHT_SIGMA, CILHIP_OPT_PLANE_WEIGHT_SIGMA, CILHIP_OPT_TILE_ACCUMULATION, CILHIP_OPT_SEARCH_DIRECTION,
  CILHIP_OPT_FEATURE_NORMAL_WEIGHT, CILHIP_OPT_FEATURE_KIND, CILHIP_OPT_FEATURE_COLOR_WEIGHT, CILHIP_OPT_SYMMETRIC_METRIC,
  CILHIP_OPT_TRANSFORM_MODE, CILHIP_OPT_REQUIRE_RECIPROCALITY, CILHIP_OPT_CELL_OCCUPANCY, CILHIP_OPT_REFINED_OCCUPANCY_FACTOR,
  CILHIP_OPT_KERNEL_TIMING, CILHIP_OPT_KERNEL_TIMING_STRIDE, CILHIP_OPT_REVERSE_WARM_START, CILHIP_OPT_FEATURE_WARM_START, CILHIP_OPT_AFFINE_DEVICE_LOOP,
  CILHIP_OPT_COUNT
} cilhip_option;
typedef struct cilhip_option_info_t {
  int id;
  const char* key;
  double default_value, min_value, max_value;
  const char* doc;
} cilhip_option_info_t;
int cilhip_option_count(void);
const cilhip_option_info_t* cilhip_option_info(int id);
int cilhip_set_option_id(cilhip_ctx* ctx, cilhip_option id, double value);
int cilhip_get_option(cilhip_ctx* ctx, const char* key, double* value);
int cilhip_get_last_timing2(cilhip_ctx* ctx, double* search_ms, double* accumulate_ms);
int cilhip_debug_counters(cilhip_ctx* ctx, uint32_t out[2]);

#ifdef __cplusplus
}
#endif
#endif
```

Baseline: 103.3 billion.

## Add tile-major target copy so LDS search tiles load cube region in one trip

After: 103.4 billion, median of 6. Within noise of the previous version (+0.1%).

```diff
diff --git a/cilantro_amd/capi.py b/cilantro_amd/capi.py
--- a/cilantro_amd/capi.py
+++ b/cilantro_amd/capi.py
@@ -18,7 +18,7 @@
     "cilhip_icp_partial_sums", "cilhip_icp_apply_sums", "cilhip_icp_state", "cilhip_compute_residuals",
     "cilhip_get_grid_info", "cilhip_get_last_timing", "cilhip_enable_kernel_timing", "cilhip_prepare_source", "cilhip_get_last_run_forms", "cilhip_get_last_warm_iterations", "cilhip_get_last_matches_origin", "cilhip_get_matches_transform", "cilhip_get_last_form_timing", "cilhip_get_last_iteration_timing", "cilhip_get_last_run_trace", "cilhip_estimate_combined_two_sets", "cilhip_icp_run_two_sets", "cilhip_set_pair_weight_callback", "cilhip_kmeans_set_pruning", "cilhip_get_tie_count", "cilhip_get_tie_rule_stats", "cilhip_get_tie_order_info", "cilhip_build_tie_order", "cilhip_tie_order_create", "cilhip_tie_order_destroy", "cilhip_tie_order_tables", "cilhip_load_tie_order", "cilhip_multi_create", "cilhip_multi_destroy", "cilhip_multi_last_error", "cilhip_multi_context", "cilhip_multi_set_clouds", "cilhip_multi_icp_run", "cilhip_multi_repartitions", "cilhip_multi_last_host_time", "cilhip_multi_set_slab_slack", "cilhip_multi_shard_sizes", "cilhip_rank_comm_unique_id", "cilhip_rank_comm_prepare", "cilhip_rank_comm_init", "cilhip_rank_comm_destroy", "cilhip_icp_iterate_ranked", "cilhip_get_last_allreduce_timing", "cilhip_get_last_host_enqueue_time", "cilhip_set_slab_guard", "cilhip_get_slab_violation", "cilhip_get_slab_violation_state",
     "cilhip_set_option", "cilhip_option_count", "cilhip_option_info", "cilhip_set_option_id", "cilhip_get_option", "cilhip_get_last_timing2", "cilhip_set_shard_info", "cilhip_icp_partial_keys",
-    "cilhip_icp_sums_from_keys", "cilhip_icp_order_keys", "cilhip_icp_sums_from_ordered_keys", "cilhip_debug_counters", "cilhip_kmeans3f", "cilhip_kmeans3f_assign", "cilhip_kmeans3f_ex", "cilhip_kmeans3f_assign_ex", "cilhip_kmeans_shard_create", "cilhip_kmeans_shard_destroy", "cilhip_kmeans_shard_maxabs", "cilhip_kmeans_scale_exponent", "cilhip_kmeans_shard_assign", "cilhip_kmeans_shard_farthest", "cilhip_kmeans_shard_move_point", "cilhip_kmeans_shard_labels",
+    "cilhip_icp_sums_from_keys", "cilhip_icp_order_keys", "cilhip_icp_sums_from_ordered_keys", "cilhip_debug_counters", "cilhip_tile_major_stats", "cilhip_kmeans3f", "cilhip_kmeans3f_assign", "cilhip_kmeans3f_ex", "cilhip_kmeans3f_assign_ex", "cilhip_kmeans_shard_create", "cilhip_kmeans_shard_destroy", "cilhip_kmeans_shard_maxabs", "cilhip_kmeans_scale_exponent", "cilhip_kmeans_shard_assign", "cilhip_kmeans_shard_farthest", "cilhip_kmeans_shard_move_point", "cilhip_kmeans_shard_labels",
     "cilhip_plane_ransac3f", "cilhip_plane_score3f", "cilhip_plane_fit3f", "cilhip_transform_ransac3f", "cilhip_transform_score3f", "cilhip_transform_fit3f", "cilhip_knn3f", "cilhip_knn_set_tie_rule", "cilhip_normals_knn3f", "cilhip_normals_radius3f", "cilhip_radius_search3f",
 ]
 
@@ -130,6 +130,7 @@
     L.cilhip_set_shard_info.argtypes = [vp, C.c_uint64, f32p, f32p]
     L.cilhip_icp_partial_keys.argtypes = [vp, vp]
     L.cilhip_debug_counters.argtypes = [vp, vp]
+    L.cilhip_tile_major_stats.argtypes = [vp, vp]
     L.cilhip_kmeans3f.argtypes = [C.c_int, f32p, C.c_size_t, C.c_int, f32p, C.c_size_t, C.c_size_t, C.c_float, vp, C.POINTER(C.c_size_t)]
     L.cilhip_kmeans3f_assign.argtypes = [C.c_int, f32p, C.c_size_t, C.c_int, f32p, C.c_size_t, vp]
     L.cilhip_kmeans3f_ex.argtypes = [C.c_int, f32p, C.c_size_t, C.c_int, f32p, C.c_size_t, C.c_size_t, C.c_float, C.c_int, vp, C.POINTER(C.c_size_t)]
diff --git a/cilantro_amd/csrc/c_api.hip b/cilantro_amd/csrc/c_api.hip
--- a/cilantro_amd/csrc/c_api.hip
+++ b/cilantro_amd/csrc/c_api.hip
@@ -39,6 +39,9 @@
   uint32_t index_offset = 0;
   bool partial_target = false;
   uint32_t* d_inv_perm = nullptr;
+  TileMajor tm{};
+  int tile_major = 1;
+  uint32_t* d_tm_count = nullptr;
 
   bool has_source = false;
   uint32_t ns = 0;
@@ -259,6 +262,7 @@
   }
   target_ptr_free(c, c->d_inv_perm); c->d_inv_perm = nullptr;
   target_ptr_free(c, c->d_safe2); c->d_safe2 = nullptr;
+  target_ptr_free(c, c->tm.cube); target_ptr_free(c, c->tm.blocks); c->tm = TileMajor();
   drop_tie_tables(c);
   drop_feat_tie_tables(c);
   release_target_share(c);
@@ -357,6 +361,7 @@
   if (c->d_winner) (void)hipFree(c->d_winner);
   if (c->d_count) (void)hipFree(c->d_count);
   if (c->d_dbg) (void)hipFree(c->d_dbg);
+  if (c->d_tm_count) (void)hipFree(c->d_tm_count);
   if (c->d_trace) (void)hipFree(c->d_trace);
   if (c->d_defer_flag) (void)hipFree(c->d_defer_flag);
   if (c->d_unproven) (void)hipFree(c->d_unproven);
@@ -426,6 +431,7 @@
   OPT(CILHIP_OPT_REVERSE_WARM_START, "reverse_warm_start", 1, 0, 1, "device-resident FIRST_TO_SECOND / BOTH loops: reverse searches after the first start from the previous reverse matches (margin test over the source; A/B)", c->reverse_warm),
   OPT(CILHIP_OPT_FEATURE_WARM_START, "feature_warm_start", 1, 0, 1, "feature adaptors (SECOND_TO_FIRST loops): searches warm-started from the previous matches once the loop moves little (margin test with the feature distance; A/B)", c->feat_warm),
   OPT(CILHIP_OPT_AFFINE_DEVICE_LOOP, "affine_device_loop", 1, 0, 1, "affine classes: 1 = device-resident loop (one-pass moments, solve in the epilogue kernel), 0 = host-driven loop (three passes + host solve; A/B)", c->affine_device_loop),
+  OPT(CILHIP_OPT_TILE_MAJOR, "tile_major", 1, 0, 1, "LDS-tiled search: a tile still on its sort-time cube copies the cube's region from a tile-major copy of the target in one trip (0: table -> scan -> staging; A/B)", c->tile_major),
 };
 #undef OPT
 constexpr int N_OPTIONS = (int)(sizeof(g_options) / sizeof(g_options[0]));
@@ -479,6 +485,11 @@
   }
   if (!strcmp(key, "pair_records")) { c->pair_records = value != 0.0; return CILHIP_OK; }
   if (!strcmp(key, "tile_records")) { c->tile_records = value != 0.0; return CILHIP_OK; }
+  if (!strcmp(key, "tile_major")) {
+    if (value != 0.0 && value != 1.0) return fail(c, CILHIP_ERR_INVALID, "tile_major: 0 or 1");
+    c->tile_major = (int)value;
+    return CILHIP_OK;
+  }
   if (!strcmp(key, "warm_enter_fraction")) {
     if (!(value > 0.0)) return fail(c, CILHIP_ERR_INVALID, "warm_enter_fraction: > 0 (fraction of a grid cell)");
     c->warm_enter = (float)value;
@@ -539,6 +550,20 @@
     return CILHIP_OK;
   }
   return fail(c, CILHIP_ERR_INVALID, "set_option: unknown key");
+}
+
+int cilhip_tile_major_stats(cilhip_ctx* c, double out[6]) {
+  if (!c || !out) return CILHIP_ERR_INVALID;
+  for (int i = 0; i < 6; ++i) out[i] = 0.0;
+  out[0] = c->tm.build_ms; out[1] = (double)c->tm.bytes; out[2] = c->tm.nblocks; out[3] = c->tm.ncubes;
+  if (!c->d_tm_count) return CILHIP_OK;
+  CK(c, hipSetDevice(c->device));
+  uint32_t h[2] = {0, 0};
+  CK(c, hipMemcpyAsync(h, c->d_tm_count, sizeof h, hipMemcpyDeviceToHost, c->stream));
+  CK(c, hipMemsetAsync(c->d_tm_count, 0, sizeof h, c->stream));
+  CK(c, hipStreamSynchronize(c->stream));
+  out[4] = h[0]; out[5] = h[1];
+  return CILHIP_OK;
 }
 
 int cilhip_debug_counters(cilhip_ctx* c, uint32_t out[2]) {
@@ -677,7 +702,8 @@
   c->dst_rgb_sorted_ok = false;
   if (!from->tshare) { from->tshare = new (std::nothrow) TargetShare(); if (!from->tshare) return fail(c, CILHIP_ERR_HIP, "share_target: out of memory"); from->tshare->refs = 1; }
   TargetShare* sh = from->tshare;
-  const void* ptrs[] = {from->grid.pts, from->grid.nrm, from->grid.pn, from->grid.cell_start, from->d_inv_perm, from->d_safe2, from->d_tie_leaf_slot, from->d_tie_nodes};
+  const void* ptrs[] = {from->grid.pts, from->grid.nrm, from->grid.pn, from->grid.cell_start, from->d_inv_perm, from->d_safe2, from->d_tie_leaf_slot, from->d_tie_nodes,
+                        from->tm.cube, from->tm.blocks};
   for (const void* p : ptrs)
     if (p && std::find(sh->allocs.begin(), sh->allocs.end(), p) == sh->allocs.end()) sh->allocs.push_back(const_cast<void*>(p));
   ++sh->refs;
@@ -687,6 +713,7 @@
   for (int i = 0; i < 3; ++i) c->dst_mean[i] = from->dst_mean[i];
   c->index_offset = from->index_offset; c->partial_target = from->partial_target;
   c->d_inv_perm = from->d_inv_perm; c->d_safe2 = from->d_safe2;
+  c->tm = from->tm; c->tm.build_ms = 0.0;
   c->d_tie_leaf_slot = from->d_tie_leaf_slot; c->d_tie_nodes = from->d_tie_nodes;
   c->warm_banned = false;
   c->src_sorted = false;
@@ -798,6 +825,14 @@
     c->d_tiles = nullptr; c->d_tile_center = nullptr; c->ntiles = 0;
     hipError_t e = sort_source(c->d_src_xyz, c->ns, c->grid, T, c->d_src_sorted, c->stream, &c->d_tiles, &c->d_tile_center, c->tile_axes, &c->ntiles, &c->sort_ws);
     if (e != hipSuccess) { c->err = std::string("sort_source: ") + hipGetErrorString(e); return CILHIP_ERR_HIP; }
+    if (c->tile_major && !c->tm.cube && c->ntiles) {
+      e = build_tile_major(c->grid, c->stream, &c->tm);
+      if (e != hipSuccess) { c->err = std::string("build_tile_major: ") + hipGetErrorString(e); return CILHIP_ERR_HIP; }
+    }
+    if (!c->d_tm_count) {
+      CK(c, hipMalloc(&c->d_tm_count, 2 * sizeof(uint32_t)));
+      CK(c, hipMemsetAsync(c->d_tm_count, 0, 2 * sizeof(uint32_t), c->stream));
+    }
     if (c->ntiles + 1 > c->tile_aux_cap) {
       if (c->d_tile_box) { (void)hipFree(c->d_tile_box); c->d_tile_box = nullptr; }
       if (c->d_defer_mask) { (void)hipFree(c->d_defer_mask); c->d_defer_mask = nullptr; }
@@ -1171,6 +1206,7 @@
   a.store_matches = 1;
   a.skip_if_inner_done = 0;
   a.tie = tie_dev_of(c);
+  if (c->tile_major && c->tm.cube) { a.tm_cube = c->tm.cube; a.tm_blocks = c->tm.blocks; a.tm_count = c->d_tm_count; }
   return a;
 }
 
diff --git a/cilantro_amd/csrc/grid_build.hip b/cilantro_amd/csrc/grid_build.hip
--- a/cilantro_amd/csrc/grid_build.hip
+++ b/cilantro_amd/csrc/grid_build.hip
@@ -315,7 +315,7 @@
                 hz = g.oz + ((float)(bz * C) + (float)GRID_PAD + 0.5f * (float)C) * g.cell;
     const float* m = Tinv.m;
     const float4 ctr = make_float4(m[0] * hx + m[4] * hy + m[8] * hz + m[12], m[1] * hx + m[5] * hy + m[9] * hz + m[13],
-                                   m[2] * hx + m[6] * hy + m[10] * hz + m[14], 0.0f);
+                                   m[2] * hx + m[6] * hy + m[10] * hz + m[14], __uint_as_float(c));
     uint32_t t = tile_off[c];
     for (uint32_t q = b; q < e; q += TILE_QUERIES) { tiles[t] = make_uint2(q, min(q + TILE_QUERIES, e)); tile_center[t] = ctr; ++t; }
   }
@@ -415,6 +415,142 @@
   return e;
 }
 
+struct TmGeom { int lo[3], RX, RY, RZ, W1, rows, E; };
+__device__ __forceinline__ TmGeom tm_geom(const GridDev& g, uint32_t c) {
+  constexpr uint32_t C = CUBE_EDGE;
+  const uint32_t cnx = (uint32_t)(g.nx - 1 - GRID_PAD) / C + 1, cny = (uint32_t)(g.ny - 1 - GRID_PAD) / C + 1;
+  int hi[3];
+  TmGeom r;
+  tm_cube_axis(c % cnx, g.nx, r.lo[0], hi[0]);
+  tm_cube_axis((c / cnx) % cny, g.ny, r.lo[1], hi[1]);
+  tm_cube_axis(c / (cnx * cny), g.nz, r.lo[2], hi[2]);
+  r.RX = hi[0] - r.lo[0] + 1; r.RY = hi[1] - r.lo[1] + 1; r.RZ = hi[2] - r.lo[2] + 1;
+  r.W1 = r.RX + 1; r.rows = r.RY * r.RZ; r.E = r.rows * r.W1;
+  return r;
+}
+__device__ __forceinline__ uint32_t tm_row_cell(const GridDev& g, const TmGeom& m, int r) {
+  const int z = r / m.RY, y = r - z * m.RY;
+  return ((uint32_t)(m.lo[2] + z) * (uint32_t)g.ny + (uint32_t)(m.lo[1] + y)) * (uint32_t)g.nx + (uint32_t)m.lo[0];
+}
+
+__global__ void k_tm_size(GridDev g, uint32_t ncubes, uint2* cube, uint32_t* size16) {
+  for (uint32_t c = blockIdx.x * blockDim.x + threadIdx.x; c < ncubes; c += gridDim.x * blockDim.x) {
+    const TmGeom m = tm_geom(g, c);
+    uint32_t P = 0;
+    for (int r = 0; r < m.rows; ++r) {
+      const uint32_t e = tm_row_cell(g, m, r);
+      P += g.cell_start[e + (uint32_t)m.RX] - g.cell_start[e];
+    }
+    const bool fits = m.RY <= TILE_MAXSPAN && m.RZ <= TILE_MAXSPAN && 4 * tm_chunks_table((uint32_t)m.E) <= (uint32_t)CILHIP_TILE_MAXE &&
+                      4 * tm_chunks_rows((uint32_t)m.rows) <= (uint32_t)TILE_MAXROWS + 1 && 4 * tm_chunks_deltas((uint32_t)m.rows) <= (uint32_t)TILE_MAXROWS &&
+                      P <= (uint32_t)TILE_CAP && 16 * tm_chunks_points(P) <= (uint32_t)TILE_BYTES;
+    cube[c] = make_uint2(NONE_U32, P);
+    size16[c] = fits ? tm_chunks_table((uint32_t)m.E) + tm_chunks_rows((uint32_t)m.rows) + tm_chunks_deltas((uint32_t)m.rows) + tm_chunks_points(P) : 0u;
+  }
+}
+
+__global__ __launch_bounds__(256) void k_tm_fill(GridDev g, uint32_t ncubes, const uint32_t* __restrict__ size16, const uint32_t* __restrict__ off,
+                                                 uint2* cube, uint4* blocks) {
+  __shared__ uint32_t fst[TILE_MAXROWS], base[TILE_MAXROWS + 1];
+  for (uint32_t c = blockIdx.x; c < ncubes; c += gridDim.x) {
+    if (size16[c] == 0) continue;
+    const TmGeom m = tm_geom(g, c);
+    uint32_t* const w = reinterpret_cast<uint32_t*>(blocks + off[c]);
+    const uint32_t n0 = tm_chunks_table((uint32_t)m.E), n1 = tm_chunks_rows((uint32_t)m.rows), n2 = tm_chunks_deltas((uint32_t)m.rows);
+    uint32_t* const wt = w;
+    uint32_t* const wb = w + 4 * n0;
+    uint32_t* const wd = wb + 4 * n1;
+    float* const wp = reinterpret_cast<float*>(wd + 4 * n2);
+    for (int e = threadIdx.x; e < 4 * (int)n0; e += blockDim.x) {
+      uint32_t v = 0;
+      if (e < m.E) { const int r = e / m.W1; v = g.cell_start[tm_row_cell(g, m, r) + (uint32_t)(e - r * m.W1)]; }
+      wt[e] = v;
+    }
+    for (int r = threadIdx.x; r < m.rows; r += blockDim.x) {
+      const uint32_t e = tm_row_cell(g, m, r);
+      fst[r] = g.cell_start[e];
+      base[r + 1] = g.cell_start[e + (uint32_t)m.RX] - fst[r];
+    }
+    __syncthreads();
+    if (threadIdx.x == 0) {
+      base[0] = 0;
+      for (int r = 0; r < m.rows; ++r) base[r + 1] += base[r];
+    }
+    __syncthreads();
+    for (int r = threadIdx.x; r < 4 * (int)n1; r += blockDim.x) wb[r] = r <= m.rows ? base[r] : 0u;
+    for (int r = threadIdx.x; r < 4 * (int)n2; r += blockDim.x) wd[r] = r < m.rows ? fst[r] - base[r] : 0u;
+    const uint32_t P = base[m.rows], npairs = (P + 11u) >> 1;
+    for (int r = threadIdx.x >> 4; r < m.rows; r += (int)(blockDim.x >> 4))
+      for (uint32_t o = threadIdx.x & 15u; o < base[r + 1] - base[r]; o += 16) {
+        const float4 q = g.pts[fst[r] + o];
+        const uint32_t j = base[r] + o;
+        float* const d = wp + (j >> 1) * 6u + (j & 1u);
+        d[0] = q.x; d[2] = q.y; d[4] = q.z;
+      }
+    for (uint32_t j = P + threadIdx.x; j < 2 * npairs; j += blockDim.x) {
+      float* const d = wp + (j >> 1) * 6u + (j & 1u);
+      d[0] = 1.0e30f; d[2] = 1.0e30f; d[4] = 1.0e30f;
+    }
+    for (uint32_t k = npairs * 6u + threadIdx.x; k < 4u * tm_chunks_points(P); k += blockDim.x) wp[k] = 0.0f;
+    if (threadIdx.x == 0) cube[c].x = off[c];
+    __syncthreads();
+  }
+}
+
+hipError_t build_tile_major(const GridDev& g, hipStream_t s, TileMajor* out) {
+  *out = TileMajor();
+  constexpr uint32_t CE = CUBE_EDGE;
+  if (g.nx <= 2 * GRID_PAD || g.ny <= 2 * GRID_PAD || g.nz <= 2 * GRID_PAD) return hipSuccess;
+  const uint32_t cnx = (uint32_t)(g.nx - 1 - GRID_PAD) / CE + 1, cny = (uint32_t)(g.ny - 1 - GRID_PAD) / CE + 1, cnz = (uint32_t)(g.nz - 1 - GRID_PAD) / CE + 1;
+  const uint32_t ncubes = cnx * cny * cnz;
+  hipEvent_t e0 = nullptr, e1 = nullptr;
+  uint32_t *size16 = nullptr, *off = nullptr;
+  void* tmp = nullptr;
+  size_t scan_tmp = 0;
+  hipError_t e = hipSuccess;
+  TileMajor t;
+  t.ncubes = ncubes;
+  do {
+    if ((e = hipEventCreate(&e0)) != hipSuccess || (e = hipEventCreate(&e1)) != hipSuccess) break;
+    if ((e = hipEventRecord(e0, s)) != hipSuccess) break;
+    if ((e = hipMalloc(&t.cube, (size_t)ncubes * sizeof(uint2))) != hipSuccess) break;
+    if ((e = hipMalloc(&size16, ((size_t)ncubes + 1) * 4)) != hipSuccess) break;
+    if ((e = hipMalloc(&off, ((size_t)ncubes + 1) * 4)) != hipSuccess) break;
+    if ((e = rocprim::exclusive_scan(nullptr, scan_tmp, size16, off, 0u, (size_t)ncubes + 1, rocprim::plus<uint32_t>(), s)) != hipSuccess) break;
+    if ((e = hipMalloc(&tmp, scan_tmp ? scan_tmp : 16)) != hipSuccess) break;
+    if ((e = hipMemsetAsync(size16 + ncubes, 0, 4, s)) != hipSuccess) break;
+    hipLaunchKernelGGL(k_tm_size, dim3(grid_blocks(ncubes)), dim3(256), 0, s, g, ncubes, t.cube, size16);
+    if ((e = rocprim::exclusive_scan(tmp, scan_tmp, size16, off, 0u, (size_t)ncubes + 1, rocprim::plus<uint32_t>(), s)) != hipSuccess) break;
+    uint32_t total16 = 0;
+    if ((e = hipMemcpyAsync(&total16, off + ncubes, 4, hipMemcpyDeviceToHost, s)) != hipSuccess) break;
+    if ((e = hipStreamSynchronize(s)) != hipSuccess) break;
+    if ((e = hipMalloc(&t.blocks, ((size_t)total16 + 1) * 16)) != hipSuccess) break;
+    hipLaunchKernelGGL(k_tm_fill, dim3(std::min(ncubes, 4096u)), dim3(256), 0, s, g, ncubes, size16, off, t.cube, t.blocks);
+    if ((e = hipGetLastError()) != hipSuccess) break;
+    std::vector<uint32_t> h(ncubes);
+    if ((e = hipMemcpyAsync(h.data(), size16, (size_t)ncubes * 4, hipMemcpyDeviceToHost, s)) != hipSuccess) break;
+    if ((e = hipEventRecord(e1, s)) != hipSuccess) break;
+    if ((e = hipEventSynchronize(e1)) != hipSuccess) break;
+    float ms = 0.f;
+    (void)hipEventElapsedTime(&ms, e0, e1);
+    t.build_ms = ms;
+    for (uint32_t v : h) t.nblocks += v != 0u;
+    t.bytes = ((size_t)total16 + 1) * 16 + (size_t)ncubes * sizeof(uint2);
+  } while (0);
+  if (size16) (void)hipFree(size16);
+  if (off) (void)hipFree(off);
+  if (tmp) (void)hipFree(tmp);
+  if (e0) (void)hipEventDestroy(e0);
+  if (e1) (void)hipEventDestroy(e1);
+  if (e != hipSuccess) {
+    if (t.cube) (void)hipFree(t.cube);
+    if (t.blocks) (void)hipFree(t.blocks);
+    return e;
+  }
+  *out = t;
+  return hipSuccess;
+}
+
 void free_sort_workspace(SortWorkspace& ws) {
   if (ws.scratch) (void)hipFree(ws.scratch);
   if (ws.tiles) (void)hipFree(ws.tiles);
diff --git a/cilantro_amd/csrc/internal.hpp b/cilantro_amd/csrc/internal.hpp
--- a/cilantro_amd/csrc/internal.hpp
+++ b/cilantro_amd/csrc/internal.hpp
@@ -149,6 +149,9 @@
   float* nn_lb;
   int lb_valid;
   TieDev tie;
+  const uint2* tm_cube;
+  const uint4* tm_blocks;
+  uint32_t* tm_count;
 };
 
 struct BoxArgs {
@@ -158,6 +161,7 @@
   uint32_t* defer_flag;
   float ox, oy, oz, inv_cell;
   int nx, ny, nz;
+  const uint2* tm_cube;
   float tile_axes[9];
   int trim;
 };
@@ -359,6 +363,24 @@
 hipError_t build_grid(const float* d_xyz, const float* d_nrm, uint32_t n, hipStream_t s,
                       GridBuildResult* out, double mean_out[3], double target_occupancy, double refined_factor = 1.0);
 void free_grid(GridDev& g);
+
+struct TileMajor {
+  uint2* cube = nullptr;
+  uint4* blocks = nullptr;
+  size_t bytes = 0;
+  uint32_t ncubes = 0, nblocks = 0;
+  double build_ms = 0.0;
+};
+__host__ __device__ inline uint32_t tm_chunks_table(uint32_t E) { return (E + 3u) >> 2; }
+__host__ __device__ inline uint32_t tm_chunks_rows(uint32_t rows) { return (rows + 4u) >> 2; }
+__host__ __device__ inline uint32_t tm_chunks_deltas(uint32_t rows) { return (rows + 3u) >> 2; }
+__host__ __device__ inline uint32_t tm_chunks_points(uint32_t P) { return (((P + 11u) >> 1) * 24u + 15u) >> 4; }
+__host__ __device__ inline void tm_cube_axis(uint32_t b, int n, int& lo, int& hi) {
+  const int c0 = GRID_PAD + (int)b * CUBE_EDGE, c1 = c0 + CUBE_EDGE - 1;
+  lo = c0 <= GRID_PAD ? 0 : c0 - 1;
+  hi = c1 >= n - 1 - GRID_PAD ? n - 1 : c1 + 1;
+}
+hipError_t build_tile_major(const GridDev& g, hipStream_t s, TileMajor* out);
 struct SortWorkspace {
   void* scratch = nullptr; size_t scratch_bytes = 0;
   uint2* tiles = nullptr; float4* centers = nullptr; uint32_t tile_cap = 0;
diff --git a/cilantro_amd/csrc/kernels.hip b/cilantro_amd/csrc/kernels.hip
--- a/cilantro_amd/csrc/kernels.hip
+++ b/cilantro_amd/csrc/kernels.hip
@@ -395,6 +395,22 @@
   const uint32_t inv_ry = RY > 0 ? (65536u + (uint32_t)RY - 1u) / (uint32_t)RY : 0u;
   int* b = g.tile_box + 8 * (size_t)t;
   b[0] = bx0; b[1] = bx1; b[2] = by0; b[3] = by1; b[4] = bz0; b[5] = bz1; b[6] = (int)inv_w1; b[7] = (int)inv_ry;
+  if (g.tm_cube != nullptr) {
+    const uint32_t cube = __float_as_uint(c4.w);
+    const uint2 cb = g.tm_cube[cube];
+    if (cb.x != NONE_U32) {
+      constexpr uint32_t C = CUBE_EDGE;
+      const uint32_t cnx = (uint32_t)(g.nx - 1 - GRID_PAD) / C + 1, cny = (uint32_t)(g.ny - 1 - GRID_PAD) / C + 1;
+      int l[3], h[3];
+      tm_cube_axis(cube % cnx, g.nx, l[0], h[0]);
+      tm_cube_axis((cube / cnx) % cny, g.ny, l[1], h[1]);
+      tm_cube_axis(cube / (cnx * cny), g.nz, l[2], h[2]);
+      bool same = true;
+#pragma unroll
+      for (int i = 0; i < 3; ++i) same = same && max(lo[i] - 1, 0) == l[i] && min(hi[i] + 1, n3[i] - 1) == h[i];
+      if (same) { b[6] = (int)(0x80000000u | cb.x); b[7] = (int)cb.y; }
+    }
+  }
 }
 
 
@@ -411,7 +427,7 @@
 
 BoxArgs make_box_args(const IterArgs& a, const float4* tile_center, int* tile_box, uint32_t ntiles, bool trim) {
   BoxArgs b{};
-  b.tile_center = tile_center; b.tile_box = tile_box; b.ntiles = ntiles; b.defer_flag = a.defer_flag;
+  b.tile_center = tile_center; b.tile_box = tile_box; b.ntiles = ntiles; b.defer_flag = a.defer_flag; b.tm_cube = a.tm_cube;
   b.ox = a.grid.ox; b.oy = a.grid.oy; b.oz = a.grid.oz; b.inv_cell = a.grid.inv_cell;
   b.nx = a.grid.nx; b.ny = a.grid.ny; b.nz = a.grid.nz;
   for (int i = 0; i < 9; ++i) b.tile_axes[i] = a.tile_axes[i];
@@ -487,6 +503,26 @@
 
   if (threadIdx.x == 0) { geom_lds[0] = lox; geom_lds[1] = loy; geom_lds[2] = loz; geom_lds[3] = RY; geom_lds[4] = W1; geom_lds[5] = rows; }
 
+  const bool tmf = tb[6] < 0;
+  if (tmf) {
+    const uint32_t Pt = (uint32_t)tb[7];
+    const uint4* const blk = a.tm_blocks + ((uint32_t)tb[6] & 0x7FFFFFFFu);
+    const uint32_t n0 = tm_chunks_table((uint32_t)E), n1 = tm_chunks_rows((uint32_t)rows), n2 = tm_chunks_deltas((uint32_t)rows), n3 = tm_chunks_points(Pt);
+    const uint32_t g0 = (n0 + 63u) >> 6, g1 = g0 + ((n1 + 63u) >> 6), g2 = g1 + ((n2 + 63u) >> 6), g3 = g2 + ((n3 + 63u) >> 6);
+    const uint32_t wave = (uint32_t)__builtin_amdgcn_readfirstlane((int)(threadIdx.x >> 6)), lane = threadIdx.x & 63u;
+    for (uint32_t gi = wave; gi < g3; gi += TILE_WAVES) {
+      uint32_t c0, n, src;
+      unsigned char* dst;
+      if (gi < g0) { c0 = gi << 6; n = n0; src = 0; dst = reinterpret_cast<unsigned char*>(lcs); }
+      else if (gi < g1) { c0 = (gi - g0) << 6; n = n1; src = n0; dst = reinterpret_cast<unsigned char*>(rowbase); }
+      else if (gi < g2) { c0 = (gi - g1) << 6; n = n2; src = n0 + n1; dst = reinterpret_cast<unsigned char*>(rowdelta); }
+      else { c0 = (gi - g2) << 6; n = n3; src = n0 + n1 + n2; dst = raw; }
+      if (c0 + lane < n)
+        __builtin_amdgcn_global_load_lds((const void*)(blk + src + c0 + lane), (__attribute__((address_space(3))) void*)(dst + 16u * c0), 16, 0, 0);
+    }
+    if (threadIdx.x == 0 && a.tm_count) atomicAdd(a.tm_count, 1u);
+  } else {
+  if (threadIdx.x == 0 && a.tm_count) atomicAdd(a.tm_count + 1, 1u);
   const __amdgpu_buffer_rsrc_t rs_cs = __builtin_amdgcn_make_buffer_rsrc(
       (void*)g.cell_start, 0, ((uint32_t)g.nx * (uint32_t)g.ny * (uint32_t)g.nz + 1u) * 4u, 0x00020000);
   {
@@ -546,6 +582,7 @@
       }
     }
     if (threadIdx.x == 63) rowbase[rows] = incl;
+  }
   }
 
   OctQuery oq[TILE_QPT];
@@ -563,6 +600,7 @@
     const bool fast = active & octant_prepare(g, qx, qy, qz, cx, cy, cz, lox, loy, loz, hix, hiy, hiz, RY, W1, oq[u]);
     flags |= (active ? (1u << u) : 0u) | (fast ? (1u << (8 + u)) : 0u);
   }
+  if (tmf) asm volatile("s_waitcnt vmcnt(0)" ::: "memory");
   __syncthreads();
   PHASE_CLK(1);
   uint32_t P = rowbase[rows];
@@ -581,7 +619,7 @@
       if ((int)floorf((oq[u].qz - g.oz) * g.inv_cell) > fz1n) flags &= ~(1u << (8 + u));
     if (threadIdx.x == 0) geom_lds[5] = rows;
   }
-  {
+  if (!tmf) {
     typedef uint32_t u32x4 __attribute__((ext_vector_type(4)));
     const __amdgpu_buffer_rsrc_t rs_pts = __builtin_amdgcn_make_buffer_rsrc((void*)g.pts, 0, g.n * 16u, 0x00020000);
     const uint32_t o0 = threadIdx.x & 15;
@@ -619,8 +657,8 @@
       for (uint32_t o = o0 + 32u; o < l; o += 16) { const float4 q = g.pts[f + o + d]; float* const w = lp + lds_slot_x(f + o); w[0] = q.x; w[2] = q.y; w[4] = q.z; }
     }
     if (threadIdx.x < 30) lp[lds_slot_x(P + threadIdx.x / 3u) + 2u * (threadIdx.x % 3u)] = 1.0e30f;
-  }
-  __syncthreads();
+    __syncthreads();
+  }
   PHASE_CLK(2);
   TileLds tl{lp, (uint32_t)reinterpret_cast<uintptr_t>(raw), (P + 1u) & ~1u, lcs, rowbase, rowdelta, lox, loy, loz, RY, W1, rows};
   uint32_t mpos[TILE_QPT];
diff --git a/cilantro_amd/icp.py b/cilantro_amd/icp.py
--- a/cilantro_amd/icp.py
+++ b/cilantro_amd/icp.py
@@ -315,6 +315,12 @@
         out = (C.c_uint32 * 2)()
         self._ck(self._L.cilhip_debug_counters(self._h, out))
         return int(out[0]), int(out[1])
+
+    def tile_major_stats(self):
+        out = (C.c_double * 6)()
+        self._ck(self._L.cilhip_tile_major_stats(self._h, out))
+        return {"build_ms": out[0], "bytes": int(out[1]), "blocks": int(out[2]), "cubes": int(out[3]),
+                "fast_tiles": int(out[4]), "fallback_tiles": int(out[5])}
 
     def set_option(self, key, value):
         self._ck(self._L.cilhip_set_option(self._h, key.encode(), float(value)))
diff --git a/include/cilantro_hip/c_api.h b/include/cilantro_hip/c_api.h
--- a/include/cilantro_hip/c_api.h
+++ b/include/cilantro_hip/c_api.h
@@ -231,7 +231,7 @@
   CILHIP_OPT_FEATURE_NORMAL_WEIGHT, CILHIP_OPT_FEATURE_KIND, CILHIP_OPT_FEATURE_COLOR_WEIGHT, CILHIP_OPT_SYMMETRIC_METRIC,
   CILHIP_OPT_TRANSFORM_MODE, CILHIP_OPT_REQUIRE_RECIPROCALITY, CILHIP_OPT_CELL_OCCUPANCY, CILHIP_OPT_REFINED_OCCUPANCY_FACTOR,
   CILHIP_OPT_KERNEL_TIMING, CILHIP_OPT_KERNEL_TIMING_STRIDE, CILHIP_OPT_REVERSE_WARM_START, CILHIP_OPT_FEATURE_WARM_START, CILHIP_OPT_AFFINE_DEVICE_LOOP,
-  CILHIP_OPT_COUNT
+  CILHIP_OPT_TILE_MAJOR, CILHIP_OPT_COUNT
 } cilhip_option;
 typedef struct cilhip_option_info_t {
   int id;
@@ -245,6 +245,7 @@
 int cilhip_get_option(cilhip_ctx* ctx, const char* key, double* value);
 int cilhip_get_last_timing2(cilhip_ctx* ctx, double* search_ms, double* accumulate_ms);
 int cilhip_debug_counters(cilhip_ctx* ctx, uint32_t out[2]);
+int cilhip_tile_major_stats(cilhip_ctx* ctx, double out[6]);
 
 #ifdef __cplusplus
 }
```
